# ramkp990/Truth_Recommendation_GNN

Measured on NVIDIA B200. Metric: message-passing edges/s (train step), higher is better.
Workload: dtype f32

## Files before the change

include/trg_b200.h:

```cpp
#ifndef TRG_B200_H
#define TRG_B200_H

#include <stddef.h>
#include <stdint.h>

#ifdef __cplusplus
extern "C" {
#endif

#define TRG_ABI_VERSION 4

enum { TRG_F32 = 0, TRG_BF16 = 1 };
enum {
  TRG_OK = 0,
  TRG_E_ARG = 1,
  TRG_E_WORKSPACE = 2,
  TRG_E_CUDA = 3,
  TRG_E_UNSUPPORTED = 4
};

int trg_abi_version(void);
const char* trg_last_error(void);
int64_t trg_launch_count(void);

size_t trg_csr_workspace_bytes(int64_t n_edges, int64_t n_key);
int trg_csr_build(const int64_t* other, const int64_t* key, int64_t n_edges, int64_t n_key,
                  int32_t* rowptr , int32_t* col , int32_t* eid ,
                  void* workspace, size_t workspace_bytes, void* stream);

size_t trg_select_range_workspace_bytes(int64_t n);
int trg_select_range(const int64_t* key, const int64_t* other, int64_t n, int64_t lo, int64_t hi,
                     int64_t capacity, int64_t pad_key, int64_t pad_other,
                     int64_t* key_out , int64_t* other_out ,
                     int32_t* count_out , void* workspace, size_t workspace_bytes, void* stream);

typedef struct {
  const int32_t* vrowptr;
  const int32_t* vinfo;
  int64_t n_vrows;
  const int32_t* long_rows;
  const int32_t* long_ptr;
  int64_t n_long;
  float* partial;
} trg_long_rows;

int trg_sage_agg_fwd(const int32_t* rowptr, const int32_t* col, const void* x_src,
                     int64_t n_dst, int32_t feat, int dtype,
                     void* mean_out , float* inv_deg_out ,
                     const trg_long_rows* long_rows , void* stream);

int trg_sage_agg_bwd(const int32_t* rowptr_t, const int32_t* col_t, const float* inv_deg,
                     const void* g_mean, int64_t n_src, int32_t feat, int dtype,
                     void* g_src_out , int out_dtype, int accumulate,
                     const void* relu_of, const trg_long_rows* long_rows ,
                     void* stream);

int trg_gather_wsum(const int32_t* rowptr, const int32_t* col, const int32_t* eid,
                    const float* coef, const float* scale, const void* x,
                    int64_t n_rows, int32_t feat, int dtype, void* out, int out_dtype, int accumulate,
                    const void* relu_of, const trg_long_rows* long_rows , void* stream);

int trg_rows_finish(const void* in, int in_dtype, const float* row_scale, const void* add,
                    const void* relu_of, int64_t n_rows, int32_t feat, int dtype, void* out, void* stream);

int trg_peer_reduce_rows(const void* const* parts, int32_t n_peers, int64_t row0, int in_dtype,
                         const float* row_scale, const void* add, const void* relu_of, int64_t n_rows,
                         int32_t feat, int dtype, void* out, int32_t ctas_per_sm, void* stream);

size_t trg_edge_bce_workspace_bytes(int64_t n_users);
int trg_edge_bce_fwd(const int32_t* rowptr_u, const int32_t* col_p, const int32_t* eid,
                     const int64_t* neg_p, const void* u, const void* p,
                     int64_t n_users, int64_t n_edges, int32_t hidden, int dtype,
                     const float* wbar , float* loss_out,
                     float* c_pos, float* c_neg, void* g_u,
                     void* workspace, size_t workspace_bytes, void* stream);

int trg_edge_anchor_loss(const int32_t* rowptr, const int32_t* col, const int32_t* eid,
                         const void* anchor, const void* gathered, int64_t n_rows,
                         int64_t n_edges_scale, int32_t hidden, int dtype, int label,
                         const float* wbar, float* loss_out, float* coef_out, void* g_anchor,
                         int accumulate, int relu_gate, void* workspace, size_t workspace_bytes,
                         void* stream);

typedef struct {
  const void* a;
  const void* w;
  int32_t k;
  float alpha;
} trg_proj_term;
size_t trg_sage_proj_workspace_bytes(int32_t k_total, int32_t hidden, int dtype);
int trg_sage_proj_fwd(const trg_proj_term* terms , int32_t n_terms,
                      const float* bias ,
                      int64_t n_rows, int32_t hidden, int dtype, int relu,
                      void* out ,
                      void* workspace, size_t workspace_bytes, void* stream);

typedef struct {
  const void* w;
  int32_t k;
  float alpha;
  const float* row_scale;
  void* d_a;
} trg_proj_bwd_term;
int trg_sage_proj_bwd_input(const void* dz, const trg_proj_bwd_term* terms , int32_t n_terms,
                            int64_t n_rows, int32_t hidden, int dtype,
                            void* workspace, size_t workspace_bytes, void* stream);

typedef struct {
  const void* a;
  int32_t k;
  float alpha;
  void* d_w;
} trg_proj_dw_term;
size_t trg_sage_proj_dw_workspace_bytes(void);
int trg_sage_proj_bwd_weight(const void* dz, const trg_proj_dw_term* terms , int32_t n_terms,
                             float* d_bias ,
                             int64_t n_rows, int32_t hidden, int dtype,
                             void* workspace, size_t workspace_bytes, void* stream);

size_t trg_score_topk_workspace_bytes(int64_t n_query, int64_t n_cat, int32_t hidden, int32_t k);
int trg_score_topk(const void* q , const void* cat ,
                   int64_t n_query, int64_t n_cat, int32_t hidden, int dtype, int32_t k,
                   int64_t id_offset, float* vals_out , int64_t* ids_out ,
                   void* workspace, size_t workspace_bytes, void* stream);
int trg_score_topk_excluding(const void* q , const void* cat ,
                             int64_t n_query, int64_t n_cat, int32_t hidden, int dtype, int32_t k,
                             int64_t id_offset, const int32_t* excl_rowptr ,
                             const int32_t* excl_ids , const int64_t* query_rows ,
                             float* vals_out , int64_t* ids_out ,
                             void* workspace, size_t workspace_bytes, void* stream);
int trg_topk_merge(const float* vals_in , const int64_t* ids_in,
                   int64_t n_query, int32_t n_lists, int32_t k_in, int32_t k_out,
                   float* vals_out, int64_t* ids_out, void* stream);

#ifdef __cplusplus
}
#endif
#endif
```

truth_recommendation_gnn_b200/_lib.py:

```python
from __future__ import annotations

import ctypes
import os

import torch

_HERE = os.path.dirname(os.path.abspath(__file__))
LIB_PATH = os.path.join(_HERE, "lib", "libtrg_b200.so")

TRG_F32, TRG_BF16 = 0, 1
ABI_VERSION = 4

_vp, _i64, _i32, _sz, _int = ctypes.c_void_p, ctypes.c_int64, ctypes.c_int32, ctypes.c_size_t, ctypes.c_int


class TrgProjTerm(ctypes.Structure):
    _fields_ = [("a", _vp), ("w", _vp), ("k", _i32), ("alpha", ctypes.c_float)]


class TrgLongRows(ctypes.Structure):
    _fields_ = [("vrowptr", _vp), ("vinfo", _vp), ("n_vrows", _i64), ("long_rows", _vp), ("long_ptr", _vp),
                ("n_long", _i64), ("partial", _vp)]


class TrgProjBwdTerm(ctypes.Structure):
    _fields_ = [("w", _vp), ("k", _i32), ("alpha", ctypes.c_float), ("row_scale", _vp), ("d_a", _vp)]


class TrgProjDwTerm(ctypes.Structure):
    _fields_ = [("a", _vp), ("k", _i32), ("alpha", ctypes.c_float), ("d_w", _vp)]


SIGNATURES = {
    "trg_abi_version": (_int, []),
    "trg_last_error": (ctypes.c_char_p, []),
    "trg_launch_count": (_i64, []),
    "trg_csr_workspace_bytes": (_sz, [_i64, _i64]),
    "trg_csr_build": (_int, [_vp, _vp, _i64, _i64, _vp, _vp, _vp, _vp, _sz, _vp]),
    "trg_select_range_workspace_bytes": (_sz, [_i64]),
    "trg_select_range": (_int, [_vp, _vp, _i64, _i64, _i64, _i64, _i64, _i64, _vp, _vp, _vp, _vp, _sz, _vp]),
    "trg_sage_agg_fwd": (_int, [_vp, _vp, _vp, _i64, _i32, _int, _vp, _vp, ctypes.POINTER(TrgLongRows), _vp]),
    "trg_sage_agg_bwd": (_int, [_vp, _vp, _vp, _vp, _i64, _i32, _int, _vp, _int, _int, _vp,
                                ctypes.POINTER(TrgLongRows), _vp]),
    "trg_gather_wsum": (_int, [_vp, _vp, _vp, _vp, _vp, _vp, _i64, _i32, _int, _vp, _int, _int, _vp,
                               ctypes.POINTER(TrgLongRows), _vp]),
    "trg_rows_finish": (_int, [_vp, _int, _vp, _vp, _vp, _i64, _i32, _int, _vp, _vp]),
    "trg_peer_reduce_rows": (_int, [_vp, _i32, _i64, _int, _vp, _vp, _vp, _i64, _i32, _int, _vp, _i32, _vp]),
    "trg_edge_bce_workspace_bytes": (_sz, [_i64]),
    "trg_edge_bce_fwd": (_int, [_vp, _vp, _vp, _vp, _vp, _vp, _i64, _i64, _i32, _int, _vp, _vp,
                                _vp, _vp, _vp, _vp, _sz, _vp]),
    "trg_edge_anchor_loss": (_int, [_vp, _vp, _vp, _vp, _vp, _i64, _i64, _i32, _int, _int, _vp, _vp, _vp,
                                    _vp, _int, _int, _vp, _sz, _vp]),
    "trg_sage_proj_workspace_bytes": (_sz, [_i32, _i32, _int]),
    "trg_sage_proj_fwd": (_int, [ctypes.POINTER(TrgProjTerm), _i32, _vp, _i64, _i32, _int, _int, _vp,
                                 _vp, _sz, _vp]),
    "trg_sage_proj_bwd_input": (_int, [_vp, ctypes.POINTER(TrgProjBwdTerm), _i32, _i64, _i32, _int,
                                       _vp, _sz, _vp]),
    "trg_sage_proj_dw_workspace_bytes": (_sz, []),
    "trg_sage_proj_bwd_weight": (_int, [_vp, ctypes.POINTER(TrgProjDwTerm), _i32, _vp, _i64, _i32, _int,
                                        _vp, _sz, _vp]),
    "trg_score_topk_workspace_bytes": (_sz, [_i64, _i64, _i32, _i32]),
    "trg_score_topk": (_int, [_vp, _vp, _i64, _i64, _i32, _int, _i32, _i64, _vp, _vp, _vp, _sz, _vp]),
    "trg_score_topk_excluding": (_int, [_vp, _vp, _i64, _i64, _i32, _int, _i32, _i64, _vp, _vp, _vp, _vp, _vp,
                                        _vp, _sz, _vp]),
    "trg_topk_merge": (_int, [_vp, _vp, _i64, _i32, _i32, _i32, _vp, _vp, _vp]),
}

_lib = None


class TrgError(RuntimeError):
    pass


def load():
    global _lib
    if _lib is None:
        if not os.path.exists(LIB_PATH):
            raise TrgError(
                f"{LIB_PATH} is missing: build it with `python -m truth_recommendation_gnn_b200.build` "
                "(nvcc, sm_100a). There is no CPU or PyTorch fallback for the hot path.")
        lib = ctypes.CDLL(LIB_PATH)
        for name, (res, args) in SIGNATURES.items():
            fn = getattr(lib, name)
            fn.restype, fn.argtypes = res, args
        if lib.trg_abi_version() != ABI_VERSION:
            raise TrgError("libtrg_b200.so ABI version mismatch; rebuild")
        _lib = lib
    return _lib


def check(rc: int, what: str):
    if rc != 0:
        raise TrgError(f"{what} failed (rc={rc}): {load().trg_last_error().decode()}")


def ptr(t):
    if t is None:
        return None
    if not t.is_cuda:
        raise TrgError("truth_recommendation_gnn_b200 runs on CUDA (sm_100a) tensors only; got a "
                       f"{t.device} tensor. There is no CPU fallback.")
    if not t.is_contiguous():
        raise TrgError("non-contiguous tensor passed to the C ABI")
    return t.data_ptr()


def stream():
    return torch.cuda.current_stream().cuda_stream


def dtype_code(dt: torch.dtype) -> int:
    if dt == torch.float32:
        return TRG_F32
    if dt == torch.bfloat16:
        return TRG_BF16
    raise TrgError(f"unsupported dtype {dt}: the hot path computes in fp32 or bf16 (fp32 accumulate)")


class Profiler:

    def __init__(self):
        self.enabled = False
        self.records = []

    def reset(self):
        self.records = []

    def summary(self):
        out = {}
        for name, nbytes, s, e in self.records:
            d = out.setdefault(name, dict(calls=0, ms=0.0, bytes=0))
            d["calls"] += 1
            d["ms"] += s.elapsed_time(e)
            d["bytes"] += int(nbytes)
        return out


PROF = Profiler()


def call(name, nbytes, fn, *args):
    if PROF.enabled:
        s, e = torch.cuda.Event(enable_timing=True), torch.cuda.Event(enable_timing=True)
        s.record()
        rc = fn(*args)
        e.record()
        PROF.records.append((name, nbytes, s, e))
    else:
        rc = fn(*args)
    check(rc, name)


def launch_count() -> int:
    return int(load().trg_launch_count())
```

truth_recommendation_gnn_b200/csrc/csr_build.cu:

```cuda
#include <algorithm>
#include <cstdio>

#include "common.cuh"

namespace trg {
namespace {

constexpr int kThreads = 256;
constexpr int kItems = 16;
constexpr int kTile = kThreads * kItems;
constexpr int kWarps = kThreads / 32;
constexpr int kRadix = 256;

template <int NWARPS>
__device__ __forceinline__ int block_exclusive_scan(int v, int* warp_sums, int& total) {
  const int lane = threadIdx.x & 31, w = threadIdx.x >> 5;
  int inc = v;
#pragma unroll
  for (int o = 1; o < 32; o <<= 1) {
    int t = __shfl_up_sync(0xffffffffu, inc, o);
    if (lane >= o) inc += t;
  }
  if (lane == 31) warp_sums[w] = inc;
  __syncthreads();
  int ws = (lane < NWARPS) ? warp_sums[lane] : 0;
  int winc = ws;
#pragma unroll
  for (int o = 1; o < NWARPS; o <<= 1) {
    int t = __shfl_up_sync(0xffffffffu, winc, o);
    if (lane >= o) winc += t;
  }
  const int wbase = __shfl_sync(0xffffffffu, winc - ws, w);
  total = __shfl_sync(0xffffffffu, winc, NWARPS - 1);
  __syncthreads();
  return wbase + inc - v;
}

__global__ void __launch_bounds__(kThreads) scan_tile_sums(const int* __restrict__ in, int64_t n,
                                                           int* __restrict__ tile_sums) {
  __shared__ int warp_sums[kWarps];
  const int64_t base = (int64_t)blockIdx.x * kTile;
  int s = 0;
#pragma unroll
  for (int i = 0; i < kItems; ++i) {
    int64_t idx = base + (int64_t)i * kThreads + threadIdx.x;
    if (idx < n) s += in[idx];
  }
  int total;
  block_exclusive_scan<kWarps>(s, warp_sums, total);
  if (threadIdx.x == 0) tile_sums[blockIdx.x] = total;
}

__global__ void __launch_bounds__(1024) scan_tile_offsets(int* __restrict__ tile_sums, int n_tiles) {
  __shared__ int warp_sums[32];
  int carry = 0;
  for (int base = 0; base < n_tiles; base += 1024) {
    int idx = base + threadIdx.x;
    int v = idx < n_tiles ? tile_sums[idx] : 0;
    int total;
    int ex = block_exclusive_scan<32>(v, warp_sums, total);
    if (idx < n_tiles) tile_sums[idx] = carry + ex;
    carry += total;
  }
}

__global__ void __launch_bounds__(kThreads) scan_apply(const int* in, int* out, int64_t n,
                                                       const int* __restrict__ tile_offsets) {
  __shared__ int warp_sums[kWarps];
  const int64_t base = (int64_t)blockIdx.x * kTile + (int64_t)threadIdx.x * kItems;
  int v[kItems];
  int s = 0;
#pragma unroll
  for (int i = 0; i < kItems; ++i) {
    v[i] = (base + i < n) ? in[base + i] : 0;
    s += v[i];
  }
  int total;
  int run = block_exclusive_scan<kWarps>(s, warp_sums, total) + tile_offsets[blockIdx.x];
#pragma unroll
  for (int i = 0; i < kItems; ++i) {
    if (base + i < n) out[base + i] = run;
    run += v[i];
  }
}

int exclusive_scan(const int* in, int* out, int64_t n, int* tile_sums, cudaStream_t st) {
  if (n <= 0) return TRG_OK;
  const int n_tiles = (int)ceil_div<int64_t>(n, kTile);
  scan_tile_sums<<<n_tiles, kThreads, 0, st>>>(in, n, tile_sums);
  scan_tile_offsets<<<1, 1024, 0, st>>>(tile_sums, n_tiles);
  scan_apply<<<n_tiles, kThreads, 0, st>>>(in, out, n, tile_sums);
  count_launch(3);
  TRG_LAUNCH_OK();
  return TRG_OK;
}

__global__ void __launch_bounds__(kThreads) count_keys(const long long* __restrict__ key, int64_t n,
                                                       long long n_key, int* __restrict__ deg) {
  int64_t i = (int64_t)blockIdx.x * blockDim.x + threadIdx.x;
  const int64_t stride = (int64_t)gridDim.x * blockDim.x;
  for (; i < n; i += stride) {
    const long long k = ldg_stream(key + i);
    if ((unsigned long long)k >= (unsigned long long)n_key) {
      printf("trg_csr_build: key %lld at edge %lld is outside [0, %lld)\n", k, (long long)i, n_key);
      __trap();
    }
    atomicAdd(&deg[(int)k], 1);
  }
}


__global__ void __launch_bounds__(kThreads) select_count(const long long* __restrict__ key, int64_t n,
                                                         long long lo, long long hi, int* __restrict__ tile_counts) {
  __shared__ int warp_sums[kWarps];
  const int64_t base = (int64_t)blockIdx.x * kTile;
  int c = 0;
#pragma unroll
  for (int i = 0; i < kItems; ++i) {
    const int64_t idx = base + (int64_t)i * kThreads + threadIdx.x;
    if (idx < n) {
      const long long k = ldg_stream(key + idx);
      c += (k >= lo && k < hi) ? 1 : 0;
    }
  }
  int total;
  block_exclusive_scan<kWarps>(c, warp_sums, total);
  if (threadIdx.x == 0) tile_counts[blockIdx.x] = total;
}

__global__ void __launch_bounds__(1024) select_offsets(int* __restrict__ tile_counts, int n_tiles,
                                                       long long capacity, int* __restrict__ count_out) {
  __shared__ int warp_sums[32];
  int carry = 0;
  for (int base = 0; base < n_tiles; base += 1024) {
    const int idx = base + threadIdx.x;
    const int v = idx < n_tiles ? tile_counts[idx] : 0;
    int total;
    const int ex = block_exclusive_scan<32>(v, warp_sums, total);
    if (idx < n_tiles) tile_counts[idx] = carry + ex;
    carry += total;
  }
  if (threadIdx.x == 0) {
    *count_out = carry;
    if ((long long)carry > capacity) {
      printf("trg_select_range: %d selected entries exceed the capacity %lld (negatives far from uniform? pass a larger "
             "capacity)\n", carry, capacity);
      __trap();
    }
  }
}

__global__ void __launch_bounds__(kThreads)
    select_scatter(const long long* __restrict__ key, const long long* __restrict__ other, int64_t n, long long lo,
                   long long hi, const int* __restrict__ tile_offsets, const int* __restrict__ count,
                   long long capacity, long long pad_key, long long pad_other, long long* __restrict__ key_out,
                   long long* __restrict__ other_out) {
  __shared__ int wtot[kWarps];
  const int lane = threadIdx.x & 31, w = threadIdx.x >> 5;
  const int64_t wbase = (int64_t)blockIdx.x * kTile + (int64_t)w * (kItems * 32);
  long long kv[kItems];
  unsigned sel[kItems];
  int mine = 0;
#pragma unroll
  for (int r = 0; r < kItems; ++r) {
    const int64_t idx = wbase + r * 32 + lane;
    kv[r] = idx < n ? ldg_stream(key + idx) : lo - 1;
    const bool in = kv[r] >= lo && kv[r] < hi;
    sel[r] = __ballot_sync(0xffffffffu, in);
    mine += __popc(sel[r]);
  }
  if (lane == 0) wtot[w] = mine;
  __syncthreads();
  int run = tile_offsets[blockIdx.x];
  for (int i = 0; i < w; ++i) run += wtot[i];
#pragma unroll
  for (int r = 0; r < kItems; ++r) {
    if ((sel[r] >> lane) & 1u) {
      const int dest = run + __popc(sel[r] & ((1u << lane) - 1u));
      if (dest < capacity) {
        key_out[dest] = kv[r] - lo;
        other_out[dest] = ldg_stream(other + wbase + r * 32 + lane);
      }
    }
    run += __popc(sel[r]);
  }
  const long long cnt = *count;
  for (long long i = cnt + (long long)blockIdx.x * kThreads + threadIdx.x; i < capacity;
       i += (long long)gridDim.x * kThreads) {
    key_out[i] = pad_key;
    other_out[i] = pad_other;
  }
}

__device__ __forceinline__ uint2 ldg_pair(const uint2* p) {
  uint2 r;
  asm volatile("ld.global.nc.L1::no_allocate.v2.u32 {%0,%1}, [%2];" : "=r"(r.x), "=r"(r.y) : "l"(p));
  return r;
}
template <bool FIRST>
__device__ __forceinline__ uint32_t load_key(const void* keys, int64_t idx) {
  if (FIRST) return (uint32_t)ldg_stream(reinterpret_cast<const long long*>(keys) + idx);
  return ldg_pair(reinterpret_cast<const uint2*>(keys) + idx).x;
}

template <bool FIRST>
__global__ void __launch_bounds__(kThreads) radix_hist(const void* __restrict__ keys, int64_t n,
                                                       int shift, int* __restrict__ hist,
                                                       int n_ctas) {
  __shared__ int h[kRadix];
  h[threadIdx.x] = 0;
  __syncthreads();
  const int64_t base = (int64_t)blockIdx.x * kTile;
#pragma unroll
  for (int i = 0; i < kItems; ++i) {
    int64_t idx = base + (int64_t)i * kThreads + threadIdx.x;
    if (idx < n) atomicAdd(&h[(load_key<FIRST>(keys, idx) >> shift) & (kRadix - 1)], 1);
  }
  __syncthreads();
  hist[(int64_t)threadIdx.x * n_ctas + blockIdx.x] = h[threadIdx.x];
}

template <bool FIRST, bool LAST>
__global__ void __launch_bounds__(kThreads)
    radix_scatter(const void* __restrict__ keys_in, int64_t n, int shift, const int* __restrict__ gbase,
                  int n_ctas, uint2* __restrict__ pairs_out, uint32_t* __restrict__ vals_out) {
  __shared__ int wcnt[kWarps][kRadix];
  __shared__ int sbase[kRadix];
  const int lane = threadIdx.x & 31, w = threadIdx.x >> 5;
#pragma unroll
  for (int i = 0; i < kWarps; ++i) wcnt[i][threadIdx.x] = 0;
  const int64_t wbase = (int64_t)blockIdx.x * kTile + (int64_t)w * (kItems * 32);

  uint32_t key[kItems], val[kItems];
#pragma unroll
  for (int r = 0; r < kItems; ++r) {
    int64_t idx = wbase + r * 32 + lane;
    bool valid = idx < n;
    if (FIRST) {
      key[r] = valid ? load_key<true>(keys_in, idx) : 0u;
      val[r] = (uint32_t)idx;
    } else {
      const uint2 kv = valid ? ldg_pair(reinterpret_cast<const uint2*>(keys_in) + idx) : make_uint2(0u, 0u);
      key[r] = kv.x;
      val[r] = kv.y;
    }
  }
  __syncthreads();

  int rank[kItems];
#pragma unroll
  for (int r = 0; r < kItems; ++r) {
    const bool valid = wbase + r * 32 + lane < n;
    const int d = valid ? (int)((key[r] >> shift) & (kRadix - 1)) : kRadix;
    const unsigned peers = __match_any_sync(0xffffffffu, d);
    const int prev = valid ? wcnt[w][d] : 0;
    __syncwarp();
    if (valid && lane == __ffs(peers) - 1) wcnt[w][d] = prev + __popc(peers);
    __syncwarp();
    rank[r] = prev + __popc(peers & ((1u << lane) - 1u));
  }
  __syncthreads();
  {
    int run = 0;
#pragma unroll
    for (int i = 0; i < kWarps; ++i) {
      int t = wcnt[i][threadIdx.x];
      wcnt[i][threadIdx.x] = run;
      run += t;
    }
    sbase[threadIdx.x] = gbase[(int64_t)threadIdx.x * n_ctas + blockIdx.x];
  }
  __syncthreads();
#pragma unroll
  for (int r = 0; r < kItems; ++r) {
    if (wbase + r * 32 + lane < n) {
      const int d = (int)((key[r] >> shift) & (kRadix - 1));
      const int dest = sbase[d] + wcnt[w][d] + rank[r];
      if (LAST)
        vals_out[dest] = val[r];
      else
        pairs_out[dest] = make_uint2(key[r], val[r]);
    }
  }
}

__global__ void __launch_bounds__(kThreads) gather_col(const long long* __restrict__ other,
                                                       const int* __restrict__ eid, int64_t n,
                                                       int* __restrict__ col) {
  int64_t i = (int64_t)blockIdx.x * blockDim.x + threadIdx.x;
  const int64_t stride = (int64_t)gridDim.x * blockDim.x;
  for (; i < n; i += stride) col[i] = (int)other[ldg_stream(eid + i)];
}

int num_passes(int64_t n_key) {
  int bits = 1;
  while (bits < 32 && ((int64_t)1 << bits) < n_key) ++bits;
  return (bits + 7) / 8;
}

struct Workspace {
  uint2* pairs[2];
  uint32_t* vals;
  int *hist, *tile_sums;
  size_t bytes;
};

Workspace carve(void* ws, int64_t e, int64_t n_key) {
  Workspace w;
  const size_t ebytes = align_up((size_t)(e > 0 ? e : 1) * 4, 256);
  const int64_t n_ctas = ceil_div<int64_t>(e > 0 ? e : 1, kTile);
  const size_t hist_bytes = align_up((size_t)kRadix * n_ctas * 4, 256);
  const int64_t scan_len = (int64_t)kRadix * n_ctas > n_key + 1 ? (int64_t)kRadix * n_ctas : n_key + 1;
  const size_t sums_bytes = align_up((size_t)ceil_div<int64_t>(scan_len, kTile) * 4 + 4, 256);
  char* p = reinterpret_cast<char*>(ws);
  w.pairs[0] = (uint2*)p; p += 2 * ebytes;
  w.pairs[1] = (uint2*)p; p += 2 * ebytes;
  w.vals = (uint32_t*)p; p += ebytes;
  w.hist = (int*)p; p += hist_bytes;
  w.tile_sums = (int*)p; p += sums_bytes;
  w.bytes = (size_t)(p - reinterpret_cast<char*>(ws));
  return w;
}

}
}

using namespace trg;

extern "C" size_t trg_csr_workspace_bytes(int64_t n_edges, int64_t n_key) {
  if (n_edges < 0 || n_key < 0) return 0;
  return carve(nullptr, n_edges, n_key).bytes;
}

extern "C" int trg_csr_build(const int64_t* other, const int64_t* key, int64_t e, int64_t n_key,
                             int32_t* rowptr, int32_t* col, int32_t* eid, void* workspace,
                             size_t workspace_bytes, void* stream) {
  cudaStream_t st = reinterpret_cast<cudaStream_t>(stream);
  TRG_CHECK_ARG(e >= 0 && n_key >= 0, "trg_csr_build: negative size");
  TRG_CHECK_ARG(e < ((int64_t)1 << 31) && n_key < ((int64_t)1 << 31) - 1,
                "trg_csr_build: n_edges=%lld / n_key=%lld exceed int32 CSR range", (long long)e,
                (long long)n_key);
  TRG_CHECK_ARG(rowptr != nullptr, "trg_csr_build: rowptr is NULL");
  TRG_CHECK_ARG(e == 0 || (key != nullptr && (col == nullptr || other != nullptr)),
                "trg_csr_build: NULL edge arrays with n_edges > 0");
  TRG_CHECK_ARG(e == 0 || n_key > 0, "trg_csr_build: edges present but n_key == 0");
  Workspace w = carve(workspace, e, n_key);
  if (workspace == nullptr || workspace_bytes < w.bytes) {
    set_error("trg_csr_build: workspace %zu < required %zu", workspace_bytes, w.bytes);
    return TRG_E_WORKSPACE;
  }
  TRG_CUDA(cudaMemsetAsync(rowptr, 0, (size_t)(n_key + 1) * sizeof(int32_t), st));
  if (e == 0) return TRG_OK;

  {
    int grid = (int)std::min<int64_t>(ceil_div<int64_t>(e, kThreads), (int64_t)kNumSMs * 16);
    count_keys<<<grid, kThreads, 0, st>>>((const long long*)key, e, (long long)n_key, rowptr);
    count_launch();
    TRG_LAUNCH_OK();
    int rc = exclusive_scan(rowptr, rowptr, n_key + 1, w.tile_sums, st);
    if (rc) return rc;
  }
  if (col == nullptr && eid == nullptr) return TRG_OK;

  const int passes = num_passes(n_key);
  const int n_ctas = (int)ceil_div<int64_t>(e, kTile);
  const void* kin = key;
  const uint32_t* vin = nullptr;
  for (int p = 0; p < passes; ++p) {
    const bool first = p == 0, last = p == passes - 1;
    const int shift = 8 * p;
    uint2* kout = w.pairs[p & 1];
    uint32_t* vout = eid ? (uint32_t*)eid : w.vals;
    if (first)
      radix_hist<true><<<n_ctas, kThreads, 0, st>>>(kin, e, shift, w.hist, n_ctas);
    else
      radix_hist<false><<<n_ctas, kThreads, 0, st>>>(kin, e, shift, w.hist, n_ctas);
    count_launch();
    TRG_LAUNCH_OK();
    int rc = exclusive_scan(w.hist, w.hist, (int64_t)kRadix * n_ctas, w.tile_sums, st);
    if (rc) return rc;
    if (first && last)
      radix_scatter<true, true><<<n_ctas, kThreads, 0, st>>>(kin, e, shift, w.hist, n_ctas, kout, vout);
    else if (first)
      radix_scatter<true, false><<<n_ctas, kThreads, 0, st>>>(kin, e, shift, w.hist, n_ctas, kout, vout);
    else if (last)
      radix_scatter<false, true><<<n_ctas, kThreads, 0, st>>>(kin, e, shift, w.hist, n_ctas, kout, vout);
    else
      radix_scatter<false, false><<<n_ctas, kThreads, 0, st>>>(kin, e, shift, w.hist, n_ctas, kout, vout);
    count_launch();
    TRG_LAUNCH_OK();
    kin = kout;
    vin = vout;
  }
  if (col != nullptr) {
    int grid = (int)std::min<int64_t>(ceil_div<int64_t>(e, kThreads), (int64_t)kNumSMs * 16);
    gather_col<<<grid, kThreads, 0, st>>>((const long long*)other, (const int*)vin, e, col);
    count_launch();
    TRG_LAUNCH_OK();
  }
  return TRG_OK;
}

extern "C" size_t trg_select_range_workspace_bytes(int64_t n) {
  if (n < 0) return 0;
  return align_up((size_t)(ceil_div<int64_t>(n > 0 ? n : 1, kTile) + 1) * 4, 256);
}

extern "C" int trg_select_range(const int64_t* key, const int64_t* other, int64_t n, int64_t lo, int64_t hi,
                                int64_t capacity, int64_t pad_key, int64_t pad_other, int64_t* key_out,
                                int64_t* other_out, int32_t* count_out, void* workspace, size_t workspace_bytes,
                                void* stream) {
  cudaStream_t st = reinterpret_cast<cudaStream_t>(stream);
  TRG_CHECK_ARG(n >= 0 && capacity >= 0 && lo <= hi, "trg_select_range: bad sizes");
  TRG_CHECK_ARG(n < ((int64_t)1 << 31) && capacity < ((int64_t)1 << 31), "trg_select_range: sizes exceed int32 range");
  TRG_CHECK_ARG(count_out && (capacity == 0 || (key_out && other_out)), "trg_select_range: NULL outputs");
  TRG_CHECK_ARG(n == 0 || (key && other), "trg_select_range: NULL inputs with n > 0");
  if (workspace == nullptr || workspace_bytes < trg_select_range_workspace_bytes(n)) {
    set_error("trg_select_range: workspace %zu < required %zu", workspace_bytes, trg_select_range_workspace_bytes(n));
    return TRG_E_WORKSPACE;
  }
  int* tile_counts = reinterpret_cast<int*>(workspace);
  const int n_tiles = (int)ceil_div<int64_t>(n > 0 ? n : 1, kTile);
  select_count<<<n_tiles, kThreads, 0, st>>>((const long long*)key, n, lo, hi, tile_counts);
  select_offsets<<<1, 1024, 0, st>>>(tile_counts, n_tiles, capacity, count_out);
  select_scatter<<<n_tiles, kThreads, 0, st>>>((const long long*)key, (const long long*)other, n, lo, hi, tile_counts,
                                               count_out, capacity, pad_key, pad_other, (long long*)key_out,
                                               (long long*)other_out);
  count_launch(3);
  TRG_LAUNCH_OK();
  return TRG_OK;
}
```

truth_recommendation_gnn_b200/csrc/edge_bce.cu:

```cuda
#include <cstdlib>

#include "common.cuh"

namespace trg {
namespace {

constexpr int kThreads = 256;

struct BceArgs {
  const int* rowptr;
  const int* col_p;
  const int* eid;
  const long long* neg_p;
  const void* u;
  const void* p;
  const float* wbar;
  float* c_pos;
  float* c_neg;
  void* g_u;
  double* partials;
  int64_t n_users;
  float inv_e;
  int row_vecs;
  int label;
  int accumulate;
  int relu_gate;
};

__device__ __forceinline__ float softplus(float x) {
  return fmaxf(x, 0.f) + log1pf(expf(-fabsf(x)));
}
__device__ __forceinline__ float sigmoid(float x) {
  const float e = expf(-fabsf(x));
  return x >= 0.f ? __fdiv_rn(1.f, 1.f + e) : __fdiv_rn(e, 1.f + e);
}

template <typename T, int LPR, int VPL, int R, bool TWO>
__global__ void __launch_bounds__(kThreads, VPL == 1 ? 3 : 2) edge_bce(const BceArgs a) {
  constexpr int kVec = Elem<T>::kVec;
  constexpr int kUnroll = (LPR < 8 ? (LPR >= 4 ? 2 : 1) : (VPL == 1 ? 4 : 2)) * (TWO ? 1 : 2);
  static_assert(R < LPR, "row boundaries are held one per lane");
  __shared__ double red[2][kThreads / 32];
  const int lane = threadIdx.x & 31;
  const int gl = lane & (LPR - 1);
  const unsigned gmask = LPR == 32 ? 0xffffffffu : (((1u << LPR) - 1u) << (lane & ~(LPR - 1)));
  const int64_t r0 = ((int64_t)blockIdx.x * (kThreads / LPR) + threadIdx.x / LPR) * R;
  const bool want_grad = a.g_u != nullptr;
  float sp_sum = 0.f, sn_sum = 0.f;

  if (r0 < a.n_users) {
    const int nr = (int)((a.n_users - r0) < (int64_t)R ? (a.n_users - r0) : (int64_t)R);
    const int my_ptr = ldg_stream(a.rowptr + r0 + min(gl, nr));
    const int e_end = __shfl_sync(gmask, my_ptr, nr, LPR);
    int e0 = __shfl_sync(gmask, my_ptr, 0, LPR);
    const size_t row_bytes = (size_t)a.row_vecs * 16;
    const char* pb = reinterpret_cast<const char*>(a.p);
    const char* ub = reinterpret_cast<const char*>(a.u);
    const float wbar = __ldg(a.wbar);

    bool act[VPL];
    float uf[VPL][kVec], ga[VPL][kVec];
    uint4 u_nxt[VPL];
#pragma unroll
    for (int i = 0; i < VPL; ++i) {
      act[i] = gl + i * LPR < a.row_vecs;
#pragma unroll
      for (int k = 0; k < kVec; ++k) uf[i][k] = ga[i][k] = 0.f;
      u_nxt[i] = make_uint4(0, 0, 0, 0);
      if (act[i]) {
        Elem<T>::unpack(ldg_row(ub + (size_t)r0 * row_bytes + (size_t)(gl + i * LPR) * 16), uf[i]);
        if (nr > 1) u_nxt[i] = ldg_row(ub + (size_t)(r0 + 1) * row_bytes + (size_t)(gl + i * LPR) * 16);
      }
    }
    int cur = 0;
    int cur_end = __shfl_sync(gmask, my_ptr, 1, LPR);

    auto flush = [&]() {
      if (want_grad) {
        char* ob = reinterpret_cast<char*>(a.g_u) + (size_t)(r0 + cur) * row_bytes;
#pragma unroll
        for (int i = 0; i < VPL; ++i)
          if (act[i]) {
            if (!TWO && a.accumulate) {
              float f[kVec];
              Elem<T>::unpack(*reinterpret_cast<const uint4*>(ob + (size_t)(gl + i * LPR) * 16), f);
#pragma unroll
              for (int k = 0; k < kVec; ++k) ga[i][k] += f[k];
            }
            if (!TWO && a.relu_gate) {
#pragma unroll
              for (int k = 0; k < kVec; ++k) ga[i][k] = uf[i][k] > 0.f ? ga[i][k] : 0.f;
            }
            stg_stream(ob + (size_t)(gl + i * LPR) * 16, Elem<T>::pack(ga[i]));
          }
      }
      ++cur;
      cur_end = __shfl_sync(gmask, my_ptr, min(cur + 1, nr), LPR);
#pragma unroll
      for (int i = 0; i < VPL; ++i) {
        Elem<T>::unpack(u_nxt[i], uf[i]);
#pragma unroll
        for (int k = 0; k < kVec; ++k) ga[i][k] = 0.f;
        if (act[i] && cur + 1 < nr)
          u_nxt[i] = ldg_row(ub + (size_t)(r0 + cur + 1) * row_bytes + (size_t)(gl + i * LPR) * 16);
      }
    };

    auto load_idx = [&](int e, int& cp, int& id) {
      cp = 0; id = 0;
      if (e < e_end) {
        cp = ldg_stream(a.col_p + e);
        id = a.eid ? ldg_stream(a.eid + e) : e;
      }
    };
    int cp_cur, id_cur, cn_cur = 0, cp_nxt, id_nxt;
    load_idx(e0 + gl, cp_cur, id_cur);
    if (TWO && e0 + gl < e_end) cn_cur = (int)ldg_stream(a.neg_p + id_cur);
    load_idx(e0 + LPR + gl, cp_nxt, id_nxt);

    while (e0 < e_end) {
      const int cnt = min(LPR, e_end - e0);
      int cn_nxt = 0;
      if (TWO && e0 + LPR + gl < e_end) cn_nxt = (int)ldg_stream(a.neg_p + id_nxt);
      int cp_nn, id_nn;
      load_idx(e0 + 2 * LPR + gl, cp_nn, id_nn);
      float my_cpos = 0.f, my_cneg = 0.f;

      int t = 0;
      while (t < cnt) {
        while (e0 + t >= cur_end) flush();
        const int bsz = min(min(kUnroll, cnt - t), cur_end - (e0 + t));
        uint4 vp[kUnroll][VPL], vn[kUnroll][VPL];
#pragma unroll
        for (int q = 0; q < kUnroll; ++q) {
          const int cpq = __shfl_sync(gmask, cp_cur, t + q, LPR);
          const int cnq = __shfl_sync(gmask, cn_cur, t + q, LPR);
          if (q < bsz) {
#pragma unroll
            for (int i = 0; i < VPL; ++i)
              if (act[i]) {
                vp[q][i] = ldg_row(pb + (size_t)cpq * row_bytes + (size_t)(gl + i * LPR) * 16);
                if (TWO) vn[q][i] = ldg_row(pb + (size_t)cnq * row_bytes + (size_t)(gl + i * LPR) * 16);
              }
          }
        }
        constexpr int NV = TWO ? 2 * kUnroll : kUnroll;
        static_assert(LPR >= NV, "transpose-reduce needs at least one lane per value");
        float v[NV];
#pragma unroll
        for (int q = 0; q < kUnroll; ++q) {
          float dp = 0.f, dn = 0.f;
          if (q < bsz) {
#pragma unroll
            for (int i = 0; i < VPL; ++i) {
              if (act[i]) {
                float fp[kVec], fn[kVec];
                Elem<T>::unpack(vp[q][i], fp);
                if (TWO) Elem<T>::unpack(vn[q][i], fn);
#pragma unroll
                for (int k = 0; k < kVec; ++k) {
                  dp = fmaf(uf[i][k], fp[k], dp);
                  if (TWO) dn = fmaf(uf[i][k], fn[k], dn);
                }
              }
            }
          }
          if (TWO) {
            v[2 * q] = dp;
            v[2 * q + 1] = dn;
          } else {
            v[q] = dp;
          }
        }
        int nv = NV;
#pragma unroll
        for (int o = LPR / 2; o > 0; o >>= 1) {
          if (nv > 1) {
            nv >>= 1;
#pragma unroll
            for (int i = 0; i < NV / 2; ++i) {
              if (i < nv) {
                const bool hi = (gl & o) != 0;
                const float send = hi ? v[i] : v[i + nv];
                const float keep = hi ? v[i + nv] : v[i];
                v[i] = keep + __shfl_xor_sync(gmask, send, o, LPR);
              }
            }
          } else {
            v[0] += __shfl_xor_sync(gmask, v[0], o, LPR);
          }
        }
        constexpr int kLanesPerVal = LPR / NV;
        const int j = gl / kLanesPerVal;
        const bool is_neg = TWO ? (j & 1) : (a.label == 0);
        const float z = is_neg ? v[0] : -v[0];
        const float spv = softplus(z);
        if ((gl % kLanesPerVal) == 0 && (TWO ? (j >> 1) : j) < bsz) {
          if (is_neg) sn_sum += spv; else sp_sum += spv;
        }
        if (want_grad) {
          const float coef = (is_neg ? 1.f : -wbar) * sigmoid(z) * a.inv_e;
#pragma unroll
          for (int q = 0; q < kUnroll; ++q) {
            const float cpos = __shfl_sync(gmask, coef, (TWO ? 2 * q : q) * kLanesPerVal, LPR);
            const float cneg = TWO ? __shfl_sync(gmask, coef, (2 * q + 1) * kLanesPerVal, LPR) : 0.f;
            if (q < bsz) {
              if (gl == t + q) {
                my_cpos = cpos;
                my_cneg = cneg;
              }
#pragma unroll
              for (int i = 0; i < VPL; ++i)
                if (act[i]) {
                  float fp[kVec], fn[kVec];
                  Elem<T>::unpack(vp[q][i], fp);
                  if (TWO) Elem<T>::unpack(vn[q][i], fn);
#pragma unroll
                  for (int k = 0; k < kVec; ++k)
                    ga[i][k] = TWO ? fmaf(cpos, fp[k], fmaf(cneg, fn[k], ga[i][k])) : fmaf(cpos, fp[k], ga[i][k]);
                }
            }
          }
        }
        t += bsz;
      }
      if (want_grad && e0 + gl < e_end) {
        a.c_pos[id_cur] = my_cpos;
        if (TWO) a.c_neg[id_cur] = my_cneg;
      }
      e0 += LPR;
      cp_cur = cp_nxt; id_cur = id_nxt; cn_cur = cn_nxt;
      cp_nxt = cp_nn; id_nxt = id_nn;
    }
    while (cur < nr) flush();
  }

  double dsp = sp_sum, dsn = sn_sum;
#pragma unroll
  for (int o = 16; o > 0; o >>= 1) {
    dsp += __shfl_xor_sync(0xffffffffu, dsp, o);
    dsn += __shfl_xor_sync(0xffffffffu, dsn, o);
  }
  if (lane == 0) {
    red[0][threadIdx.x >> 5] = dsp;
    red[1][threadIdx.x >> 5] = dsn;
  }
  __syncthreads();
  if (threadIdx.x == 0) {
    double s0 = 0, s1 = 0;
#pragma unroll
    for (int w = 0; w < kThreads / 32; ++w) {
      s0 += red[0][w];
      s1 += red[1][w];
    }
    a.partials[2 * (size_t)blockIdx.x] = s0;
    a.partials[2 * (size_t)blockIdx.x + 1] = s1;
  }
}

__device__ __forceinline__ void cp_async16(uint32_t dst, const void* src) {
  asm volatile("cp.async.cg.shared.global [%0], [%1], 16;" ::"r"(dst), "l"(src) : "memory");
}
__device__ __forceinline__ void cp_async_commit() { asm volatile("cp.async.commit_group;" ::: "memory"); }
template <int N>
__device__ __forceinline__ void cp_async_wait() {
  asm volatile("cp.async.wait_group %0;" ::"n"(N) : "memory");
}
__device__ __forceinline__ uint4 lds128_bce(uint32_t addr) {
  uint4 v;
  asm volatile("ld.shared.v4.u32 {%0,%1,%2,%3}, [%4];" : "=r"(v.x), "=r"(v.y), "=r"(v.z), "=r"(v.w) : "r"(addr) : "memory");
  return v;
}

constexpr int kRingG = 8;
constexpr int kRingS = 16;
constexpr int kRingBytes = (kThreads / 32) * kRingS * 512;

template <typename T>
__global__ void __launch_bounds__(kThreads, 3) edge_anchor_ring(const BceArgs a) {
  constexpr int kVec = Elem<T>::kVec;
  constexpr int R = 4, G = kRingG, S = kRingS;
  constexpr unsigned full = 0xffffffffu;
  extern __shared__ __align__(16) unsigned char ring_raw[];
  __shared__ double red[2][kThreads / 32];
  const int lane = threadIdx.x & 31, warp = threadIdx.x >> 5;
  const uint32_t ring_a = static_cast<uint32_t>(__cvta_generic_to_shared(ring_raw)) +
                          (uint32_t)(warp * S * 512 + lane * 16);
  const int64_t r0 = ((int64_t)blockIdx.x * (kThreads / 32) + warp) * R;
  const bool want_grad = a.g_u != nullptr;
  float s_sum = 0.f;

  if (r0 < a.n_users) {
    const int nr = (int)((a.n_users - r0) < (int64_t)R ? (a.n_users - r0) : (int64_t)R);
    const int my_ptr = ldg_stream(a.rowptr + r0 + min(lane, nr));
    const int e_end = __shfl_sync(full, my_ptr, nr);
    const int e_beg = __shfl_sync(full, my_ptr, 0);
    const char* pb = reinterpret_cast<const char*>(a.p);
    const char* ub = reinterpret_cast<const char*>(a.u);
    const float wbar = __ldg(a.wbar);
    const bool is_neg = a.label == 0;

    float uf[kVec], ga[kVec];
    uint4 u_nxt = make_uint4(0, 0, 0, 0);
#pragma unroll
    for (int k = 0; k < kVec; ++k) ga[k] = 0.f;
    Elem<T>::unpack(ldg_row(ub + (size_t)r0 * 512 + (size_t)lane * 16), uf);
    if (nr > 1) u_nxt = ldg_row(ub + (size_t)(r0 + 1) * 512 + (size_t)lane * 16);
    int cur = 0;
    int cur_end = __shfl_sync(full, my_ptr, 1);

    auto flush = [&]() {
      if (want_grad) {
        char* ob = reinterpret_cast<char*>(a.g_u) + (size_t)(r0 + cur) * 512 + (size_t)lane * 16;
        if (a.accumulate) {
          float f[kVec];
          Elem<T>::unpack(*reinterpret_cast<const uint4*>(ob), f);
#pragma unroll
          for (int k = 0; k < kVec; ++k) ga[k] += f[k];
        }
        if (a.relu_gate) {
#pragma unroll
          for (int k = 0; k < kVec; ++k) ga[k] = uf[k] > 0.f ? ga[k] : 0.f;
        }
        stg_stream(ob, Elem<T>::pack(ga));
      }
      ++cur;
      cur_end = __shfl_sync(full, my_ptr, min(cur + 1, nr));
      Elem<T>::unpack(u_nxt, uf);
#pragma unroll
      for (int k = 0; k < kVec; ++k) ga[k] = 0.f;
      if (cur + 1 < nr) u_nxt = ldg_row(ub + (size_t)(r0 + cur + 1) * 512 + (size_t)lane * 16);
    };
    auto load_id = [&](int ebase) -> int {
      const int e = ebase + lane;
      return (lane < G && e < e_end) ? ldg_stream(a.col_p + e) : 0;
    };
    auto issue = [&](int ebase, int ids, int slot0) {
#pragma unroll
      for (int q = 0; q < G; ++q) {
        const int rid = __shfl_sync(full, ids, q);
        if (ebase + q < e_end)
          cp_async16(ring_a + (uint32_t)(((slot0 + q) & (S - 1)) * 512), pb + (size_t)rid * 512 + (size_t)lane * 16);
      }
      cp_async_commit();
    };

    {
      const int id0 = load_id(e_beg), id1 = load_id(e_beg + G);
      issue(e_beg, id0, 0);
      issue(e_beg + G, id1, G);
    }
    int nid = load_id(e_beg + 2 * G);
    int slot = 0;
    for (int e_base = e_beg; e_base < e_end; e_base += G) {
      const int cnt = min(G, e_end - e_base);
      int my_id = 0;
      if (want_grad && lane < cnt) my_id = a.eid ? ldg_stream(a.eid + e_base + lane) : e_base + lane;
      cp_async_wait<1>();
      __syncwarp();
      float my_c = 0.f;
      int t = 0;
      while (t < cnt) {
        while (e_base + t >= cur_end) flush();
        const int bsz = min(cnt - t, cur_end - (e_base + t));
        uint4 vp[G];
        float v[G];
#pragma unroll
        for (int q = 0; q < G; ++q) {
          float dp = 0.f;
          if (q < bsz) {
            vp[q] = lds128_bce(ring_a + (uint32_t)(((slot + t + q) & (S - 1)) * 512));
            float fp[kVec];
            Elem<T>::unpack(vp[q], fp);
#pragma unroll
            for (int k = 0; k < kVec; ++k) dp = fmaf(uf[k], fp[k], dp);
          }
          v[q] = dp;
        }
        int nv = G;
#pragma unroll
        for (int o = 16; o > 0; o >>= 1) {
          if (nv > 1) {
            nv >>= 1;
#pragma unroll
            for (int i = 0; i < G / 2; ++i) {
              if (i < nv) {
                const bool hi = (lane & o) != 0;
                const float send = hi ? v[i] : v[i + nv];
                const float keep = hi ? v[i + nv] : v[i];
                v[i] = keep + __shfl_xor_sync(full, send, o);
              }
            }
          } else {
            v[0] += __shfl_xor_sync(full, v[0], o);
          }
        }
        constexpr int kLanesPerVal = 32 / G;
        const int j = lane / kLanesPerVal;
        const float z = is_neg ? v[0] : -v[0];
        const float spv = softplus(z);
        if ((lane % kLanesPerVal) == 0 && j < bsz) s_sum += spv;
        if (want_grad) {
          const float coef = (is_neg ? 1.f : -wbar) * sigmoid(z) * a.inv_e;
#pragma unroll
          for (int q = 0; q < G; ++q) {
            const float cq = __shfl_sync(full, coef, q * kLanesPerVal);
            if (q < bsz) {
              if (lane == t + q) my_c = cq;
              float fp[kVec];
              Elem<T>::unpack(vp[q], fp);
#pragma unroll
              for (int k = 0; k < kVec; ++k) ga[k] = fmaf(cq, fp[k], ga[k]);
            }
          }
        }
        t += bsz;
      }
      if (want_grad && lane < cnt) a.c_pos[my_id] = my_c;
      __syncwarp();
      const int nid_next = load_id(e_base + 3 * G);
      issue(e_base + 2 * G, nid, slot);
      nid = nid_next;
      slot = (slot + G) & (S - 1);
    }
    while (cur < nr) flush();
    cp_async_wait<0>();
  }

  double dsum = s_sum;
#pragma unroll
  for (int o = 16; o > 0; o >>= 1) dsum += __shfl_xor_sync(0xffffffffu, dsum, o);
  if (lane == 0) red[0][warp] = dsum;
  __syncthreads();
  if (threadIdx.x == 0) {
    double s0 = 0;
#pragma unroll
    for (int w = 0; w < kThreads / 32; ++w) s0 += red[0][w];
    const bool neg = a.label == 0;
    a.partials[2 * (size_t)blockIdx.x] = neg ? 0.0 : s0;
    a.partials[2 * (size_t)blockIdx.x + 1] = neg ? s0 : 0.0;
  }
}

__global__ void __launch_bounds__(1024) edge_bce_finish(const double* __restrict__ partials,
                                                        int64_t n_parts, const float* wbar,
                                                        double n_edges, float* loss_out) {
  __shared__ double red[2][32];
  double s0 = 0, s1 = 0;
  for (int64_t i = threadIdx.x; i < n_parts; i += 1024) {
    s0 += partials[2 * i];
    s1 += partials[2 * i + 1];
  }
#pragma unroll
  for (int o = 16; o > 0; o >>= 1) {
    s0 += __shfl_xor_sync(0xffffffffu, s0, o);
    s1 += __shfl_xor_sync(0xffffffffu, s1, o);
  }
  if ((threadIdx.x & 31) == 0) {
    red[0][threadIdx.x >> 5] = s0;
    red[1][threadIdx.x >> 5] = s1;
  }
  __syncthreads();
  if (threadIdx.x == 0) {
    s0 = s1 = 0;
    for (int w = 0; w < 32; ++w) {
      s0 += red[0][w];
      s1 += red[1][w];
    }
    const float pos_loss = (float)(s0 / n_edges);
    const float neg_loss = (float)(s1 / n_edges);
    loss_out[0] = __ldg(wbar) * pos_loss + neg_loss;
  }
}

template <typename T, bool TWO>
int launch_bce(BceArgs& a, int64_t* n_blocks_out, cudaStream_t st, bool dry) {
  const int rv = a.row_vecs;
#define TRG_BCE_CASE(LPR, VPL, R)                                                     \
  {                                                                                   \
    const int64_t grid = ceil_div<int64_t>(a.n_users, (int64_t)(kThreads / LPR) * R); \
    *n_blocks_out = grid;                                                             \
    if (!dry) edge_bce<T, LPR, VPL, R, TWO><<<(unsigned)grid, kThreads, 0, st>>>(a);  \
  }
  if (rv <= 2) TRG_BCE_CASE(2, 1, 1)
  else if (rv <= 4) TRG_BCE_CASE(4, 1, 2)
  else if (rv <= 8) TRG_BCE_CASE(8, 1, 4)
  else if (rv <= 16) TRG_BCE_CASE(16, 1, 4)
  else if (rv <= 32) TRG_BCE_CASE(32, 1, 4)
  else if (rv <= 64) TRG_BCE_CASE(32, 2, 4)
  else {
    set_error("trg_edge_bce_fwd: rows wider than 1024 bytes are not supported (row_vecs=%d)", rv);
    return TRG_E_UNSUPPORTED;
  }
#undef TRG_BCE_CASE
  return TRG_OK;
}

}
}

using namespace trg;

static bool anchor_ring_off() { return debug_env_int("TRG_K4_RING", 1) == 0; }

extern "C" size_t trg_edge_bce_workspace_bytes(int64_t n_users) {
  if (n_users < 0) return 0;
  return align_up((size_t)(ceil_div<int64_t>(n_users, 8) + 1) * 16, 256);
}

extern "C" int trg_edge_bce_fwd(const int32_t* rowptr_u, const int32_t* col_p, const int32_t* eid,
                                const int64_t* neg_p, const void* u, const void* p, int64_t n_users,
                                int64_t n_edges, int32_t hidden, int dtype, const float* wbar,
                                float* loss_out, float* c_pos, float* c_neg, void* g_u,
                                void* workspace, size_t workspace_bytes, void* stream) {
  cudaStream_t st = reinterpret_cast<cudaStream_t>(stream);
  TRG_CHECK_ARG(n_users >= 0 && n_edges >= 0, "trg_edge_bce_fwd: negative size");
  TRG_CHECK_ARG(loss_out && wbar, "trg_edge_bce_fwd: NULL loss_out/wbar");
  TRG_CHECK_ARG((c_pos == nullptr) == (g_u == nullptr) && (c_neg == nullptr) == (g_u == nullptr),
                "trg_edge_bce_fwd: c_pos, c_neg and g_u must be all NULL or all non-NULL");
  TRG_CHECK_ARG(n_users == 0 || (rowptr_u && u && p), "trg_edge_bce_fwd: NULL rowptr / tables");
  TRG_CHECK_ARG(((uintptr_t)u | (uintptr_t)p | (uintptr_t)g_u) % 16 == 0,
                "trg_edge_bce_fwd: tables must be 16-byte aligned");
  const int es = dtype == TRG_BF16 ? 2 : 4;
  TRG_CHECK_ARG(dtype == TRG_F32 || dtype == TRG_BF16, "trg_edge_bce_fwd: unknown dtype %d", dtype);
  TRG_CHECK_ARG(hidden > 0 && (hidden * es) % 16 == 0,
                "trg_edge_bce_fwd: row width %d x %d bytes is not a multiple of 16 bytes", hidden, es);
  if (workspace == nullptr || workspace_bytes < trg_edge_bce_workspace_bytes(n_users)) {
    set_error("trg_edge_bce_fwd: workspace %zu < required %zu", workspace_bytes,
              trg_edge_bce_workspace_bytes(n_users));
    return TRG_E_WORKSPACE;
  }
  BceArgs a{};
  a.rowptr = rowptr_u; a.col_p = col_p; a.eid = eid; a.neg_p = (const long long*)neg_p;
  a.u = u; a.p = p; a.wbar = wbar; a.c_pos = c_pos; a.c_neg = c_neg; a.g_u = g_u;
  a.partials = reinterpret_cast<double*>(workspace);
  a.n_users = n_users;
  a.inv_e = n_edges > 0 ? (float)(1.0 / (double)n_edges) : 0.f;
  a.row_vecs = hidden * es / 16;
  int64_t n_blocks = 0;
  if (n_users > 0) {
    int rc = dtype == TRG_F32 ? launch_bce<float, true>(a, &n_blocks, st, false)
                              : launch_bce<__nv_bfloat16, true>(a, &n_blocks, st, false);
    if (rc) return rc;
    count_launch();
    TRG_LAUNCH_OK();
  }
  edge_bce_finish<<<1, 1024, 0, st>>>(a.partials, n_blocks, wbar, (double)n_edges, loss_out);
  count_launch();
  TRG_LAUNCH_OK();
  return TRG_OK;
}

extern "C" int trg_edge_anchor_loss(const int32_t* rowptr, const int32_t* col, const int32_t* eid,
                                    const void* anchor, const void* gathered, int64_t n_rows,
                                    int64_t n_edges_scale, int32_t hidden, int dtype, int label,
                                    const float* wbar, float* loss_out, float* coef_out, void* g_anchor,
                                    int accumulate, int relu_gate, void* workspace, size_t workspace_bytes,
                                    void* stream) {
  cudaStream_t st = reinterpret_cast<cudaStream_t>(stream);
  TRG_CHECK_ARG(n_rows >= 0 && n_edges_scale >= 0, "trg_edge_anchor_loss: negative size");
  TRG_CHECK_ARG(loss_out && wbar, "trg_edge_anchor_loss: NULL loss_out/wbar");
  TRG_CHECK_ARG((coef_out == nullptr) == (g_anchor == nullptr),
                "trg_edge_anchor_loss: coef_out and g_anchor must be both NULL or both non-NULL");
  TRG_CHECK_ARG(n_rows == 0 || (rowptr && anchor), "trg_edge_anchor_loss: NULL rowptr / anchor table");
  TRG_CHECK_ARG(((uintptr_t)anchor | (uintptr_t)gathered | (uintptr_t)g_anchor) % 16 == 0,
                "trg_edge_anchor_loss: tables must be 16-byte aligned");
  TRG_CHECK_ARG(dtype == TRG_F32 || dtype == TRG_BF16, "trg_edge_anchor_loss: unknown dtype %d", dtype);
  const int es = dtype == TRG_BF16 ? 2 : 4;
  TRG_CHECK_ARG(hidden > 0 && (hidden * es) % 16 == 0,
                "trg_edge_anchor_loss: row width %d x %d bytes is not a multiple of 16 bytes", hidden, es);
  if (workspace == nullptr || workspace_bytes < trg_edge_bce_workspace_bytes(n_rows)) {
    set_error("trg_edge_anchor_loss: workspace %zu < required %zu", workspace_bytes,
              trg_edge_bce_workspace_bytes(n_rows));
    return TRG_E_WORKSPACE;
  }
  BceArgs a{};
  a.rowptr = rowptr; a.col_p = col; a.eid = eid; a.neg_p = nullptr;
  a.u = anchor; a.p = gathered; a.wbar = wbar; a.c_pos = coef_out; a.c_neg = nullptr; a.g_u = g_anchor;
  a.partials = reinterpret_cast<double*>(workspace);
  a.n_users = n_rows;
  a.inv_e = n_edges_scale > 0 ? (float)(1.0 / (double)n_edges_scale) : 0.f;
  a.row_vecs = hidden * es / 16;
  a.label = label ? 1 : 0;
  a.accumulate = accumulate ? 1 : 0;
  a.relu_gate = relu_gate ? 1 : 0;
  int64_t n_blocks = 0;
  if (n_rows > 0 && a.row_vecs == 32 && !anchor_ring_off()) {
    n_blocks = ceil_div<int64_t>(n_rows, (int64_t)(kThreads / 32) * 4);
    static SmemAttrState attr_f32, attr_bf16;
    if (dtype == TRG_F32) {
      TRG_CUDA(ensure_dyn_smem(edge_anchor_ring<float>, kRingBytes, attr_f32));
      edge_anchor_ring<float><<<(unsigned)n_blocks, kThreads, kRingBytes, st>>>(a);
    } else {
      TRG_CUDA(ensure_dyn_smem(edge_anchor_ring<__nv_bfloat16>, kRingBytes, attr_bf16));
      edge_anchor_ring<__nv_bfloat16><<<(unsigned)n_blocks, kThreads, kRingBytes, st>>>(a);
    }
    count_launch();
    TRG_LAUNCH_OK();
  } else if (n_rows > 0) {
    int rc = dtype == TRG_F32 ? launch_bce<float, false>(a, &n_blocks, st, false)
                              : launch_bce<__nv_bfloat16, false>(a, &n_blocks, st, false);
    if (rc) return rc;
    count_launch();
    TRG_LAUNCH_OK();
  }
  edge_bce_finish<<<1, 1024, 0, st>>>(a.partials, n_blocks, wbar, (double)n_edges_scale, loss_out);
  count_launch();
  TRG_LAUNCH_OK();
  return TRG_OK;
}
```

truth_recommendation_gnn_b200/functional.py:

```python
from __future__ import annotations

import ctypes

import torch

from . import _lib
from .graph import CSR, RelationGraph, build_csr


def _long_rows_arg(csr: CSR, feat: int, dev, elem_size: int = 4):
    lr = csr.long_rows() if feat * elem_size >= 80 else None
    if lr is None:
        return None, None
    partial = torch.empty(lr.n_slots, feat, dtype=torch.float32, device=dev)
    s = _lib.TrgLongRows(_lib.ptr(lr.vrowptr), _lib.ptr(lr.vinfo), int(lr.vinfo.numel()), _lib.ptr(lr.long_rows),
                         _lib.ptr(lr.long_ptr), int(lr.long_rows.numel()), _lib.ptr(partial))
    return ctypes.byref(s), (s, partial)


def _check_rows(x: torch.Tensor, what: str):
    es = x.element_size()
    if x.dim() != 2 or (x.size(1) * es) % 16 != 0:
        raise _lib.TrgError(f"{what}: rows must be a multiple of 16 bytes (got shape {tuple(x.shape)}, "
                            f"{x.dtype}); pad the feature width (the reference pads to 64, inference.py:401-404)")


def sage_agg_fwd(csr: CSR, x_src: torch.Tensor, want_inv_deg: bool = True):
    lib = _lib.load()
    _check_rows(x_src, "sage_agg_fwd")
    x_src = x_src.contiguous()
    out = torch.empty(csr.n_rows, x_src.size(1), dtype=x_src.dtype, device=x_src.device)
    inv_deg = torch.empty(csr.n_rows, dtype=torch.float32, device=x_src.device) if want_inv_deg else None
    if csr.n_rows:
        rb = x_src.size(1) * x_src.element_size()
        nbytes = csr.n_edges * (rb + 4) + 4 * (csr.n_rows + 1) + csr.n_rows * rb
        lr, keep = _long_rows_arg(csr, x_src.size(1), x_src.device, x_src.element_size())
        _lib.call("trg_sage_agg_fwd", nbytes, lib.trg_sage_agg_fwd,
                  _lib.ptr(csr.rowptr), _lib.ptr(csr.col), _lib.ptr(x_src), csr.n_rows, x_src.size(1),
                  _lib.dtype_code(x_src.dtype), _lib.ptr(out), _lib.ptr(inv_deg), lr, _lib.stream())
    return out, inv_deg


def _check_epilogue(out, relu_of, n_rows, x, who, out_dtype=None):
    for t, what, dt in ((out, "out", out_dtype or x.dtype), (relu_of, "relu_of", x.dtype)):
        if t is not None and (t.shape != (n_rows, x.size(1)) or t.dtype != dt or not t.is_contiguous()
                              or t.device != x.device):
            raise _lib.TrgError(f"{who}: {what} must be a contiguous [{n_rows}, {x.size(1)}] {dt} tensor")


def _out_dtype(x, out, out_dtype):
    if out_dtype is None:
        out_dtype = out.dtype if out is not None else x.dtype
    if out_dtype != x.dtype and not (x.dtype == torch.bfloat16 and out_dtype == torch.float32):
        raise _lib.TrgError(f"output dtype {out_dtype} is not supported for a {x.dtype} table")
    return out_dtype


def sage_agg_bwd(csr_t: CSR, inv_deg, g_mean: torch.Tensor, out=None, accumulate=False, relu_of=None,
                 out_dtype=None):
    lib = _lib.load()
    g_mean = g_mean.contiguous()
    _check_rows(g_mean, "sage_agg_bwd")
    out_dtype = _out_dtype(g_mean, out, out_dtype)
    _check_epilogue(out, relu_of, csr_t.n_rows, g_mean, "sage_agg_bwd", out_dtype)
    if out is None:
        out = torch.empty(csr_t.n_rows, g_mean.size(1), dtype=out_dtype, device=g_mean.device)
        accumulate = False
    if csr_t.n_rows:
        rb = g_mean.size(1) * g_mean.element_size()
        ob = g_mean.size(1) * out.element_size()
        nbytes = (csr_t.n_edges * (rb + 4) + 4 * (csr_t.n_rows + 1)
                  + csr_t.n_rows * (ob * (1 + bool(accumulate)) + rb * (relu_of is not None))
                  + (4 * csr_t.n_cols if inv_deg is not None else 0))
        lr, keep = _long_rows_arg(csr_t, g_mean.size(1), g_mean.device, g_mean.element_size())
        _lib.call("trg_sage_agg_bwd", nbytes, lib.trg_sage_agg_bwd,
                  _lib.ptr(csr_t.rowptr), _lib.ptr(csr_t.col), _lib.ptr(inv_deg), _lib.ptr(g_mean),
                  csr_t.n_rows, g_mean.size(1), _lib.dtype_code(g_mean.dtype), _lib.ptr(out),
                  _lib.dtype_code(out_dtype), 1 if accumulate else 0, _lib.ptr(relu_of), lr, _lib.stream())
    return out


class SageAggFn(torch.autograd.Function):

    @staticmethod
    def forward(ctx, x_src, rel: RelationGraph, grad_prescaled: bool = False):
        want_inv = rel.inv_deg is None
        mean, inv_deg = sage_agg_fwd(rel.fwd, x_src, want_inv_deg=want_inv)
        if want_inv:
            rel.inv_deg = inv_deg
        ctx.rel = rel
        ctx.grad_prescaled = grad_prescaled
        return mean

    @staticmethod
    def backward(ctx, g_mean):
        if not ctx.needs_input_grad[0]:
            return None, None, None
        rel = ctx.rel
        return sage_agg_bwd(rel.bwd, None if ctx.grad_prescaled else rel.inv_deg, g_mean), None, None


def sage_mean_aggregate(x_src: torch.Tensor, rel: RelationGraph, grad_prescaled: bool = False) -> torch.Tensor:
    return SageAggFn.apply(x_src, rel, grad_prescaled)


def gather_wsum(csr: CSR, coef, x: torch.Tensor, scale=None, out=None, accumulate=False, relu_of=None,
                out_dtype=None):
    lib = _lib.load()
    x = x.contiguous()
    _check_rows(x, "gather_wsum")
    out_dtype = _out_dtype(x, out, out_dtype)
    _check_epilogue(out, relu_of, csr.n_rows, x, "gather_wsum", out_dtype)
    if out is None:
        out = torch.empty(csr.n_rows, x.size(1), dtype=out_dtype, device=x.device)
        accumulate = False
    if csr.n_rows:
        rb = x.size(1) * x.element_size()
        ob = x.size(1) * out.element_size()
        nbytes = (csr.n_edges * (rb + 12) + 4 * (csr.n_rows + 1)
                  + csr.n_rows * (ob * (1 + bool(accumulate)) + rb * (relu_of is not None)))
        lr, keep = _long_rows_arg(csr, x.size(1), x.device, x.element_size())
        _lib.call("trg_gather_wsum", nbytes, lib.trg_gather_wsum,
                  _lib.ptr(csr.rowptr), _lib.ptr(csr.col), _lib.ptr(csr.eid), _lib.ptr(coef),
                  _lib.ptr(scale), _lib.ptr(x), csr.n_rows, x.size(1), _lib.dtype_code(x.dtype),
                  _lib.ptr(out), _lib.dtype_code(out_dtype), 1 if accumulate else 0, _lib.ptr(relu_of), lr,
                  _lib.stream())
    return out


def rows_finish(x, dtype, row_scale=None, add=None, relu_of=None, out=None):
    lib = _lib.load()
    x = x.contiguous()
    n, feat = x.shape
    if x.dtype != dtype and x.dtype != torch.float32:
        raise _lib.TrgError(f"rows_finish: input must be {dtype} or float32, got {x.dtype}")
    for t, what in ((add, "add"), (relu_of, "relu_of"), (out, "out")):
        if t is not None and (t.shape != x.shape or t.dtype != dtype or not t.is_contiguous()):
            raise _lib.TrgError(f"rows_finish: {what} must be a contiguous [{n}, {feat}] {dtype} tensor")
    if out is None:
        out = torch.empty(n, feat, dtype=dtype, device=x.device)
    _check_rows(out, "rows_finish")
    rs = row_scale.float().contiguous() if row_scale is not None else None
    es = out.element_size()
    nbytes = n * feat * (x.element_size() + es * (1 + (add is not None) + (relu_of is not None)))
    _lib.call("trg_rows_finish", nbytes, lib.trg_rows_finish, _lib.ptr(x), _lib.dtype_code(x.dtype), _lib.ptr(rs),
              _lib.ptr(add), _lib.ptr(relu_of), n, feat, _lib.dtype_code(dtype), _lib.ptr(out), _lib.stream())
    return out


def peer_reduce_rows(parts, row0, n_rows, dtype, row_scale=None, add=None, relu_of=None, ctas_per_sm=0):
    import ctypes
    lib = _lib.load()
    feat = parts[0].size(1)
    for t in parts:
        if t.dtype != parts[0].dtype or t.size(1) != feat or t.size(0) < row0 + n_rows or not t.is_contiguous():
            raise _lib.TrgError("peer_reduce_rows: partial tables must be contiguous, of one dtype and width, and "
                                "hold rows [row0, row0 + n_rows)")
    if parts[0].dtype != dtype and parts[0].dtype != torch.float32:
        raise _lib.TrgError(f"peer_reduce_rows: partial tables must be {dtype} or float32")
    for t, what in ((add, "add"), (relu_of, "relu_of")):
        if t is not None and (tuple(t.shape) != (n_rows, feat) or t.dtype != dtype or not t.is_contiguous()):
            raise _lib.TrgError(f"peer_reduce_rows: {what} must be a contiguous [{n_rows}, {feat}] {dtype} tensor")
    out = torch.empty(n_rows, feat, dtype=dtype, device=parts[0].device)
    _check_rows(out, "peer_reduce_rows")
    rs = row_scale.float().contiguous() if row_scale is not None else None
    ptrs = (ctypes.c_void_p * len(parts))(*[_lib.ptr(t) for t in parts])
    nbytes = n_rows * feat * (len(parts) * parts[0].element_size()
                              + out.element_size() * (1 + (add is not None) + (relu_of is not None)))
    _lib.call("trg_peer_reduce_rows", nbytes, lib.trg_peer_reduce_rows, ptrs, len(parts), row0,
              _lib.dtype_code(parts[0].dtype), _lib.ptr(rs), _lib.ptr(add), _lib.ptr(relu_of), n_rows, feat,
              _lib.dtype_code(dtype), _lib.ptr(out), ctas_per_sm, _lib.stream())
    return out


class LinkStructure:

    def __init__(self, train_edge_index, interaction_type_tensor, num_users, num_posts):
        pos_u, pos_p = train_edge_index[0], train_edge_index[1]
        self.train_edge_index = train_edge_index
        self.num_users, self.num_posts = int(num_users), int(num_posts)
        self.n_edges = int(pos_u.numel())
        self.by_user = build_csr(pos_p, pos_u, self.num_users, self.num_posts)
        self.by_post = build_csr(pos_u, pos_p, self.num_posts, self.num_users, validate=False)
        self._by_post_u = None
        self._user_of_u = None
        if self.n_edges:
            w = interaction_type_tensor[pos_p + num_users].float()
            self.wbar = w.mean().reshape(1).contiguous()
        else:
            self.wbar = torch.full((1,), float("nan"), device=pos_u.device)


    @property
    def by_post_u(self) -> CSR:
        if self._by_post_u is None:
            bu, bp = self.by_user, self.by_post
            inv = torch.empty(self.n_edges, dtype=torch.int32, device=bu.eid.device)
            inv[bu.eid.long()] = torch.arange(self.n_edges, dtype=torch.int32, device=bu.eid.device)
            self._by_post_u = CSR(bp.rowptr, bp.col, inv[bp.eid.long()].contiguous(), bp.n_rows, bp.n_cols, bp._long)
        return self._by_post_u

    @property
    def user_of_u(self) -> torch.Tensor:
        if self._user_of_u is None:
            rp = self.by_user.rowptr.long()
            self._user_of_u = torch.repeat_interleave(
                torch.arange(self.num_users, device=rp.device), rp[1:] - rp[:-1]).contiguous()
        return self._user_of_u


_LINK_CACHE: dict = {}


def link_structure(train_edge_index, interaction_type_tensor, num_users, num_posts) -> LinkStructure:
    key = (train_edge_index.data_ptr(), tuple(train_edge_index.shape), train_edge_index._version,
           interaction_type_tensor.data_ptr(), interaction_type_tensor._version, int(num_users),
           int(num_posts))
    s = _LINK_CACHE.get(key)
    if s is None:
        if len(_LINK_CACHE) > 8:
            _LINK_CACHE.clear()
        s = LinkStructure(train_edge_index, interaction_type_tensor, num_users, num_posts)
        s._keepalive = interaction_type_tensor
        _LINK_CACHE[key] = s
    return s


def edge_bce_fwd(ls: LinkStructure, user_emb, post_emb, neg_p, want_grad: bool):
    lib = _lib.load()
    _check_rows(user_emb, "edge_bce_fwd")
    if user_emb.dtype != post_emb.dtype or user_emb.size(1) != post_emb.size(1):
        raise _lib.TrgError("user and post embeddings must share dtype and width")
    if neg_p.dtype != torch.int64 or neg_p.numel() != ls.n_edges:
        raise _lib.TrgError("neg_p must be int64 with one entry per positive edge (train_gnn.py:272)")
    user_emb, post_emb, neg_p = user_emb.contiguous(), post_emb.contiguous(), neg_p.contiguous()
    dev = user_emb.device
    loss = torch.empty(1, dtype=torch.float32, device=dev)
    c_pos = c_neg = g_u = None
    if want_grad:
        c_pos = torch.empty(ls.n_edges, dtype=torch.float32, device=dev)
        c_neg = torch.empty(ls.n_edges, dtype=torch.float32, device=dev)
        g_u = torch.empty_like(user_emb)
    ws_bytes = int(lib.trg_edge_bce_workspace_bytes(ls.num_users))
    ws = torch.empty(ws_bytes, dtype=torch.uint8, device=dev)
    e = ls.n_edges
    e_scale = int(getattr(ls, "n_edges_scale", e))
    rb = user_emb.size(1) * user_emb.element_size()
    nbytes = e * (2 * rb + 16 + (8 if want_grad else 0)) + ls.num_users * (rb * (2 if want_grad else 1) + 4)
    _lib.call("trg_edge_bce_fwd", nbytes, lib.trg_edge_bce_fwd,
              _lib.ptr(ls.by_user.rowptr), _lib.ptr(ls.by_user.col) if e else None,
              _lib.ptr(ls.by_user.eid) if e else None, _lib.ptr(neg_p) if e else None,
              _lib.ptr(user_emb), _lib.ptr(post_emb), ls.num_users, e_scale, user_emb.size(1),
              _lib.dtype_code(user_emb.dtype), _lib.ptr(ls.wbar), _lib.ptr(loss), _lib.ptr(c_pos),
              _lib.ptr(c_neg), _lib.ptr(g_u), _lib.ptr(ws), ws_bytes, _lib.stream())
    return loss, c_pos, c_neg, g_u


def edge_anchor_loss(csr: CSR, anchor, gathered, n_edges_scale, label, wbar, want_grad, g_anchor=None,
                     relu_gate=False, coef_in_csr_order=False):
    lib = _lib.load()
    anchor, gathered = anchor.contiguous(), gathered.contiguous()
    _check_rows(anchor, "edge_anchor_loss")
    dev = anchor.device
    loss = torch.empty(1, dtype=torch.float32, device=dev)
    coef = None
    accumulate = g_anchor is not None
    if want_grad:
        coef = torch.empty(csr.n_edges, dtype=torch.float32, device=dev)
        if g_anchor is None:
            g_anchor = torch.empty_like(anchor)
    else:
        g_anchor = None
    ws_bytes = int(lib.trg_edge_bce_workspace_bytes(csr.n_rows))
    ws = torch.empty(ws_bytes, dtype=torch.uint8, device=dev)
    e = csr.n_edges
    rb = anchor.size(1) * anchor.element_size()
    nbytes = e * (rb + 12) + csr.n_rows * (rb * (2 if want_grad else 1) + 4)
    _lib.call("trg_edge_anchor_loss", nbytes, lib.trg_edge_anchor_loss,
              _lib.ptr(csr.rowptr), _lib.ptr(csr.col) if e else None,
              _lib.ptr(csr.eid) if (e and not coef_in_csr_order) else None,
              _lib.ptr(anchor), _lib.ptr(gathered), csr.n_rows, int(n_edges_scale), anchor.size(1),
              _lib.dtype_code(anchor.dtype), 1 if label else 0, _lib.ptr(wbar), _lib.ptr(loss), _lib.ptr(coef),
              _lib.ptr(g_anchor), 1 if (accumulate and want_grad) else 0,
              1 if (relu_gate and want_grad) else 0, _lib.ptr(ws), ws_bytes, _lib.stream())
    return loss, coef, g_anchor


class LinkBCEFn(torch.autograd.Function):

    @staticmethod
    def forward(ctx, user_emb, post_emb, neg_p, ls: LinkStructure):
        want = user_emb.requires_grad or post_emb.requires_grad
        if neg_p.dtype != torch.int64 or neg_p.numel() != ls.n_edges:
            raise _lib.TrgError("neg_p must be int64 with one entry per positive edge (train_gnn.py:272)")
        if getattr(ls, "eid_long", None) is None:
            ls.eid_long = ls.by_user.eid.long()
        e_scale = int(getattr(ls, "n_edges_scale", ls.n_edges))
        bu = ls.by_user
        ctx.neg_by_post = None
        if want and ls.n_edges:
            ctx.neg_by_post = build_csr(ls.train_edge_index[0], neg_p, ls.num_posts, ls.num_users, validate=False,
                                        per_step=True)
        col_neg = neg_p.index_select(0, ls.eid_long).int()
        neg_csr = CSR(bu.rowptr, col_neg, bu.eid, bu.n_rows, bu.n_cols)
        l_pos, c_pos, g_u = edge_anchor_loss(bu, user_emb, post_emb, e_scale, 1, ls.wbar, want, None)
        l_neg, c_neg, g_u = edge_anchor_loss(neg_csr, user_emb, post_emb, e_scale, 0, ls.wbar, want, g_u)
        ctx.ls = ls
        ctx.want = want
        if want:
            ctx.save_for_backward(user_emb, neg_p, c_pos, c_neg, g_u)
        return (l_pos + l_neg).reshape(())

    @staticmethod
    def backward(ctx, g):
        user_emb, neg_p, c_pos, c_neg, g_u = ctx.saved_tensors
        ls = ctx.ls
        g = g.reshape(1).float().contiguous()
        g_user = g_post = None
        if ctx.needs_input_grad[0]:
            g_user = g_u * g.to(g_u.dtype)
        if ctx.needs_input_grad[1]:
            g_post = gather_wsum(ls.by_post, c_pos, user_emb, scale=g)
            if ctx.neg_by_post is not None:
                gather_wsum(ctx.neg_by_post, c_neg, user_emb, scale=g, out=g_post, accumulate=True)
        return g_user, g_post, None, None


def link_bce_loss(user_emb, post_emb, train_edge_index, neg_p, interaction_type_tensor, num_users):
    ls = link_structure(train_edge_index, interaction_type_tensor, num_users, post_emb.size(0))
    return LinkBCEFn.apply(user_emb, post_emb, neg_p, ls)


def _proj_bytes(n, ks, hidden, es):
    return n * (sum(ks) + hidden) * es


def sage_proj_fwd(terms, bias, relu: bool):
    lib = _lib.load()
    a0 = terms[0][0]
    n, hidden = a0.size(0), terms[0][1].size(0)
    arr = (_lib.TrgProjTerm * len(terms))()
    keep = []
    for i, (a, w, alpha) in enumerate(terms):
        a, w = a.contiguous(), w.contiguous()
        if a.dtype != a0.dtype or w.dtype != a0.dtype:
            raise _lib.TrgError("projection operands must share one dtype")
        keep += [a, w]
        arr[i].a, arr[i].w, arr[i].k, arr[i].alpha = _lib.ptr(a), _lib.ptr(w), a.size(1), float(alpha)
    out = torch.empty(n, hidden, dtype=a0.dtype, device=a0.device)
    b = bias.float().contiguous() if bias is not None else None
    ktot = sum(t[0].size(1) for t in terms)
    code = _lib.dtype_code(a0.dtype)
    ws_bytes = int(lib.trg_sage_proj_workspace_bytes(ktot, hidden, code))
    ws = torch.empty(ws_bytes, dtype=torch.uint8, device=a0.device)
    _lib.call("trg_sage_proj_fwd", _proj_bytes(n, [t[0].size(1) for t in terms], hidden, a0.element_size()),
              lib.trg_sage_proj_fwd, arr, len(terms), _lib.ptr(b), n, hidden, code, 1 if relu else 0,
              _lib.ptr(out), _lib.ptr(ws), ws_bytes, _lib.stream())
    return out


def sage_proj_bwd_input(dz, terms):
    lib = _lib.load()
    dz = dz.contiguous()
    n, hidden = dz.shape
    arr = (_lib.TrgProjBwdTerm * len(terms))()
    outs, keep = [], []
    for i, (w, alpha, rs) in enumerate(terms):
        w = w.contiguous()
        if w.dtype != dz.dtype:
            raise _lib.TrgError("projection operands must share one dtype")
        d_a = torch.empty(n, w.size(1), dtype=dz.dtype, device=dz.device)
        rs = rs.float().contiguous() if rs is not None else None
        keep += [w, rs]
        outs.append(d_a)
        arr[i].w, arr[i].k, arr[i].alpha = _lib.ptr(w), w.size(1), float(alpha)
        arr[i].row_scale, arr[i].d_a = _lib.ptr(rs), _lib.ptr(d_a)
    ktot = sum(t[0].size(1) for t in terms)
    code = _lib.dtype_code(dz.dtype)
    ws_bytes = int(lib.trg_sage_proj_workspace_bytes(ktot, hidden, code))
    ws = torch.empty(ws_bytes, dtype=torch.uint8, device=dz.device)
    _lib.call("trg_sage_proj_bwd_input", n * (len(terms) * hidden + ktot) * dz.element_size(),
              lib.trg_sage_proj_bwd_input, _lib.ptr(dz), arr, len(terms), n, hidden, code,
              _lib.ptr(ws), ws_bytes, _lib.stream())
    return outs


class FusedProjFn(torch.autograd.Function):

    @staticmethod
    def forward(ctx, relu, alphas, row_scales, bias, *aw):
        n_t = len(aw) // 2
        a_list, w_list = aw[:n_t], aw[n_t:]
        out = sage_proj_fwd([(a, w, al) for a, w, al in zip(a_list, w_list, alphas)], bias, relu)
        ctx.relu, ctx.alphas, ctx.row_scales, ctx.n_t = relu, alphas, row_scales, n_t
        ctx.has_bias = bias is not None
        ctx.bias_dtype = bias.dtype if bias is not None else None
        ctx.save_for_backward(out, *a_list, *w_list)
        return out

    @staticmethod
    def backward(ctx, g):
        out, *rest = ctx.saved_tensors
        n_t = ctx.n_t
        a_list, w_list = rest[:n_t], rest[n_t:]
        g = g.contiguous()
        dz = torch.ops.aten.threshold_backward(g, out, 0) if ctx.relu else g
        need_a = [ctx.needs_input_grad[4 + t] for t in range(n_t)]
        need_w = [ctx.needs_input_grad[4 + n_t + t] for t in range(n_t)]
        d_a = [None] * n_t
        idx = [t for t in range(n_t) if need_a[t]]
        if idx:
            outs = sage_proj_bwd_input(dz, [(w_list[t], ctx.alphas[t], ctx.row_scales[t]) for t in idx])
            for t, o in zip(idx, outs):
                d_a[t] = o
        d_w = [None] * n_t
        widx = [t for t in range(n_t) if need_w[t]]
        want_b = ctx.has_bias and ctx.needs_input_grad[3]
        d_b = None
        if widx or want_b:
            outs, d_b = sage_proj_bwd_weight(dz, [(a_list[t], ctx.alphas[t]) for t in widx], want_b)
            for t, o in zip(widx, outs):
                d_w[t] = o
            if d_b is not None:
                d_b = d_b.to(ctx.bias_dtype)
        return (None, None, None, d_b, *d_a, *d_w)


def sage_proj_bwd_weight(dz, terms, want_bias: bool):
    lib = _lib.load()
    dz = dz.contiguous()
    n, hidden = dz.shape
    arr = (_lib.TrgProjDwTerm * max(len(terms), 1))()
    outs, keep = [], []
    for i, (a, alpha) in enumerate(terms):
        a = a.contiguous()
        d_w = torch.empty(hidden, a.size(1), dtype=dz.dtype, device=dz.device)
        keep.append(a)
        outs.append(d_w)
        arr[i].a, arr[i].k, arr[i].alpha, arr[i].d_w = _lib.ptr(a), a.size(1), float(alpha), _lib.ptr(d_w)
    db = torch.empty(hidden, dtype=torch.float32, device=dz.device) if want_bias else None
    ws_bytes = int(lib.trg_sage_proj_dw_workspace_bytes())
    ws = torch.empty(ws_bytes, dtype=torch.uint8, device=dz.device)
    ktot = sum(t[0].size(1) for t in terms)
    _lib.call("trg_sage_proj_bwd_weight", n * (hidden + ktot) * dz.element_size(),
              lib.trg_sage_proj_bwd_weight, _lib.ptr(dz), arr, len(terms), _lib.ptr(db), n, hidden,
              _lib.dtype_code(dz.dtype), _lib.ptr(ws), ws_bytes, _lib.stream())
    return outs, db


def fused_projection(terms, bias, relu=True, row_scales=None):
    a_list = [t[0] for t in terms]
    w_list = [t[1] for t in terms]
    alphas = tuple(float(t[2]) for t in terms)
    rs = tuple(row_scales) if row_scales is not None else (None,) * len(terms)
    return FusedProjFn.apply(relu, alphas, rs, bias, *a_list, *w_list)


def score_topk(q: torch.Tensor, cat: torch.Tensor, k: int, id_offset: int = 0, exclude=None, rows=None):
    lib = _lib.load()
    if q.dim() == 1:
        q = q.unsqueeze(0)
    q, cat = q.contiguous(), cat.contiguous()
    b, h = q.shape
    p = cat.size(0)
    kk = min(int(k), p)
    if exclude is None and rows is not None:
        raise ValueError("score_topk: rows selects exclusion rows and needs exclude")
    if exclude is not None:
        if rows is None:
            if b > exclude.num_rows:
                raise ValueError(f"score_topk: {b} queries but the exclusion index has {exclude.num_rows} rows; "
                                 "pass rows= to map queries to rows")
        else:
            if rows.dtype != torch.int64 or rows.dim() != 1 or rows.numel() != b:
                raise ValueError(f"score_topk: rows must be int64 [B={b}]")
            rows = rows.contiguous()
    vals = torch.empty(b, kk, dtype=torch.float32, device=q.device)
    ids = torch.empty(b, kk, dtype=torch.int64, device=q.device)
    if b == 0 or kk == 0:
        return vals, ids
    ws_bytes = int(lib.trg_score_topk_workspace_bytes(b, p, h, kk))
    ws = torch.empty(ws_bytes, dtype=torch.uint8, device=q.device)
    if exclude is None:
        _lib.call("trg_score_topk", 2 * b * p * h, lib.trg_score_topk,
                  _lib.ptr(q), _lib.ptr(cat), b, p, h, _lib.dtype_code(q.dtype), kk, int(id_offset),
                  _lib.ptr(vals), _lib.ptr(ids), _lib.ptr(ws), ws_bytes, _lib.stream())
    else:
        _lib.call("trg_score_topk_excluding", 2 * b * p * h, lib.trg_score_topk_excluding,
                  _lib.ptr(q), _lib.ptr(cat), b, p, h, _lib.dtype_code(q.dtype), kk, int(id_offset),
                  _lib.ptr(exclude.rowptr), _lib.ptr(exclude.ids if exclude.nnz else exclude.rowptr), _lib.ptr(rows),
                  _lib.ptr(vals), _lib.ptr(ids), _lib.ptr(ws), ws_bytes, _lib.stream())
    return vals, ids


def topk_merge(vals_in: torch.Tensor, ids_in: torch.Tensor, n_lists: int, k_out: int):
    lib = _lib.load()
    b = vals_in.size(0)
    k_in = vals_in.size(1) // n_lists
    vals = torch.empty(b, k_out, dtype=torch.float32, device=vals_in.device)
    ids = torch.empty(b, k_out, dtype=torch.int64, device=vals_in.device)
    _lib.check(lib.trg_topk_merge(_lib.ptr(vals_in.contiguous()), _lib.ptr(ids_in.contiguous()), b,
                                  n_lists, k_in, k_out, _lib.ptr(vals), _lib.ptr(ids), _lib.stream()),
               "trg_topk_merge")
    return vals, ids
```

truth_recommendation_gnn_b200/fused_step.py:

```python
from __future__ import annotations

import torch

from . import _lib
from .functional import (edge_anchor_loss, gather_wsum, link_structure, sage_agg_bwd, sage_agg_fwd,
                         sage_proj_bwd_input, sage_proj_bwd_weight, sage_proj_fwd)
from .graph import CSR, build_csr, relation_graph
from .nn import REL_DIRECT, REL_ENGAGE, REL_SOCIAL, StackedWeightedRGCN, WeightedRGCN


def _layers(model):
    if type(model) is StackedWeightedRGCN:
        return list(model.layers)
    if type(model) is WeightedRGCN:
        return [model]
    return None


def eligible(model, x_dict) -> bool:
    layers = _layers(model)
    if layers is None or not torch.is_grad_enabled():
        return False
    xu, xp = x_dict["user"], x_dict["post"]
    if not (xu.is_cuda and xp.is_cuda) or xu.requires_grad or xp.requires_grad or xu.dtype != xp.dtype:
        return False
    for layer in layers:
        for conv in (layer.msg_direct, layer.msg_social, layer.post_update):
            if conv.lin_l.bias is None:
                return False
    return all(p.requires_grad for p in model.parameters())


def _accum(param, grad):
    grad = grad.to(param.dtype)
    if param.grad is None:
        param.grad = grad
    else:
        param.grad.add_(grad)


def _agg(rel, x):
    want_inv = rel.inv_deg is None
    mean, inv_deg = sage_agg_fwd(rel.fwd, x, want_inv_deg=want_inv)
    if want_inv:
        rel.inv_deg = inv_deg
    return mean


@torch.no_grad()
def loss_and_grads(model, x_dict, edge_index_dict, train_edge_index, interaction_type_tensor, num_users,
                   neg_p, neg_ready=None):
    layers = _layers(model)
    if layers is None:
        raise _lib.TrgError("loss_and_grads: model must be WeightedRGCN or StackedWeightedRGCN")
    hu, hp = x_dict["user"].contiguous(), x_dict["post"].contiguous()
    n_u, n_p = hu.size(0), hp.size(0)
    rel_d = relation_graph(edge_index_dict[REL_DIRECT], n_p, n_u)
    rel_s = relation_graph(edge_index_dict[REL_SOCIAL], n_u, n_u)
    rel_e = relation_graph(edge_index_dict[REL_ENGAGE], n_u, n_p)

    saved = []
    for layer in layers:
        d, s, p = layer.msg_direct, layer.msg_social, layer.post_update
        for conv, (xs, xd) in ((d, (hp, hu)), (s, (hu, hu)), (p, (hu, hp))):
            conv.lin_l.materialize(xs.size(-1))
            conv.lin_r.materialize(xd.size(-1))
        wd, ws = float(layer.w_direct), float(layer.w_social)
        mean_d, mean_s, mean_e = _agg(rel_d, hp), _agg(rel_s, hu), _agg(rel_e, hu)
        w_root = wd * d.lin_r.weight + ws * s.lin_r.weight
        b_user = wd * d.lin_l.bias + ws * s.lin_l.bias
        hu_n = sage_proj_fwd([(mean_d, d.lin_l.weight, wd), (mean_s, s.lin_l.weight, ws), (hu, w_root, 1.0)],
                             b_user, True)
        hp_n = sage_proj_fwd([(mean_e, p.lin_l.weight, 1.0), (hp, p.lin_r.weight, 1.0)], p.lin_l.bias, True)
        saved.append((hu, hp, mean_d, mean_s, mean_e, w_root))
        hu, hp = hu_n, hp_n

    ls = link_structure(train_edge_index, interaction_type_tensor, num_users, n_p)
    if neg_ready is not None:
        torch.cuda.current_stream().wait_event(neg_ready)
    if neg_p.dtype != torch.int64 or neg_p.numel() != ls.n_edges:
        raise _lib.TrgError("neg_p must be int64 with one entry per positive edge (train_gnn.py:272)")
    if getattr(ls, "eid_long", None) is None:
        ls.eid_long = ls.by_user.eid.long()
    bu = ls.by_user
    col_neg64 = neg_p.index_select(0, ls.eid_long)
    neg_by_post = build_csr(ls.user_of_u, col_neg64, n_p, n_u, validate=False, per_step=True)
    neg_by_user = CSR(bu.rowptr, col_neg64.int(), bu.eid, bu.n_rows, bu.n_cols)
    l_pos, c_pos, dz_u = edge_anchor_loss(bu, hu, hp, ls.n_edges, 1, ls.wbar, True, None, coef_in_csr_order=True)
    l_neg, c_neg, dz_u = edge_anchor_loss(neg_by_user, hu, hp, ls.n_edges, 0, ls.wbar, True, dz_u,
                                          relu_gate=True, coef_in_csr_order=True)
    dz_p = gather_wsum(ls.by_post_u, c_pos, hu)
    gather_wsum(neg_by_post, c_neg, hu, out=dz_p, accumulate=True, relu_of=hp)
    del col_neg64
    loss = (l_pos + l_neg).reshape(())
    del neg_by_user, neg_by_post, c_pos, c_neg, hu, hp

    for li in range(len(layers) - 1, -1, -1):
        layer = layers[li]
        d, s, p = layer.msg_direct, layer.msg_social, layer.post_update
        wd, ws = float(layer.w_direct), float(layer.w_social)
        hu_in, hp_in, mean_d, mean_s, mean_e, w_root = saved.pop()
        (dw_d, dw_s, dw_root), db_u = sage_proj_bwd_weight(dz_u, [(mean_d, wd), (mean_s, ws), (hu_in, 1.0)], True)
        (dw_p, dw_pr), db_p = sage_proj_bwd_weight(dz_p, [(mean_e, 1.0), (hp_in, 1.0)], True)
        del mean_d, mean_s, mean_e
        _accum(d.lin_l.weight, dw_d)
        _accum(s.lin_l.weight, dw_s)
        _accum(d.lin_r.weight, wd * dw_root)
        _accum(s.lin_r.weight, ws * dw_root)
        _accum(d.lin_l.bias, wd * db_u)
        _accum(s.lin_l.bias, ws * db_u)
        _accum(p.lin_l.weight, dw_p)
        _accum(p.lin_r.weight, dw_pr)
        _accum(p.lin_l.bias, db_p)
        if li == 0:
            break
        g_md, g_ms, g_hu = sage_proj_bwd_input(
            dz_u, [(d.lin_l.weight, wd, rel_d.inv_deg), (s.lin_l.weight, ws, rel_s.inv_deg), (w_root, 1.0, None)])
        g_me, g_hp = sage_proj_bwd_input(dz_p, [(p.lin_l.weight, 1.0, rel_e.inv_deg), (p.lin_r.weight, 1.0, None)])
        del dz_u, dz_p
        sage_agg_bwd(rel_s.bwd, None, g_ms, out=g_hu, accumulate=True)
        sage_agg_bwd(rel_e.bwd, None, g_me, out=g_hu, accumulate=True, relu_of=hu_in)
        sage_agg_bwd(rel_d.bwd, None, g_md, out=g_hp, accumulate=True, relu_of=hp_in)
        dz_u, dz_p = g_hu, g_hp
    return loss
```

Baseline: 2.965 billion.

## Fuse negative-sample CSR build and post-side loss gradient into merged kernels

Replaces the per-step int64 index_select plus full CSR build for negative edges with a dedicated kernel that gathers negatives as int32, counts post degrees, and radix-sorts with an int32 key path. Positive and negative edges are merged into one by-post CSR. A new post-side edge kernel then recomputes the edge gradients directly instead of storing per-edge coefficients and running two gather_wsum passes. This cuts launches and coefficient traffic, at the cost of recomputing dot products on the post side and only applying when rows are 512 bytes wide.

```diff
diff --git a/include/trg_b200.h b/include/trg_b200.h
--- a/include/trg_b200.h
+++ b/include/trg_b200.h
@@ -8,7 +8,7 @@
 extern "C" {
 #endif
 
-#define TRG_ABI_VERSION 4
+#define TRG_ABI_VERSION 5
 
 enum { TRG_F32 = 0, TRG_BF16 = 1 };
 enum {
@@ -27,6 +27,13 @@
 int trg_csr_build(const int64_t* other, const int64_t* key, int64_t n_edges, int64_t n_key,
                   int32_t* rowptr , int32_t* col , int32_t* eid ,
                   void* workspace, size_t workspace_bytes, void* stream);
+
+size_t trg_loss_negatives_workspace_bytes(int64_t n_edges, int64_t n_posts);
+int trg_loss_negatives(const int64_t* neg_p, const int32_t* eid_u, const int32_t* user_of_u, int64_t n_edges,
+                       int64_t n_posts, const int32_t* rowptr_post, const int32_t* col_post,
+                       const int32_t* post_of_pos, const int32_t* rowptr_pos, const int32_t* vrow, int64_t n_rows,
+                       int32_t* col_neg , int32_t* rowptr_m , int32_t* col_m ,
+                       void* workspace, size_t workspace_bytes, void* stream);
 
 size_t trg_select_range_workspace_bytes(int64_t n);
 int trg_select_range(const int64_t* key, const int64_t* other, int64_t n, int64_t lo, int64_t hi,
@@ -81,6 +88,12 @@
                          const float* wbar, float* loss_out, float* coef_out, void* g_anchor,
                          int accumulate, int relu_gate, void* workspace, size_t workspace_bytes,
                          void* stream);
+
+int trg_edge_post_grad(const int32_t* rowptr, const int32_t* rowptr_pos, const int32_t* col, const int32_t* vrow,
+                       const int32_t* vinfo, const void* anchor, const void* gathered, int64_t n_rows,
+                       int64_t n_edges_scale, int32_t hidden, int dtype, const float* wbar, void* g_anchor,
+                       int relu_gate, const int32_t* long_rows, const int32_t* long_ptr, int64_t n_long,
+                       int64_t n_slots, float* partial, void* stream);
 
 typedef struct {
   const void* a;
diff --git a/truth_recommendation_gnn_b200/_lib.py b/truth_recommendation_gnn_b200/_lib.py
--- a/truth_recommendation_gnn_b200/_lib.py
+++ b/truth_recommendation_gnn_b200/_lib.py
@@ -9,7 +9,7 @@
 LIB_PATH = os.path.join(_HERE, "lib", "libtrg_b200.so")
 
 TRG_F32, TRG_BF16 = 0, 1
-ABI_VERSION = 4
+ABI_VERSION = 5
 
 _vp, _i64, _i32, _sz, _int = ctypes.c_void_p, ctypes.c_int64, ctypes.c_int32, ctypes.c_size_t, ctypes.c_int
 
@@ -37,6 +37,9 @@
     "trg_launch_count": (_i64, []),
     "trg_csr_workspace_bytes": (_sz, [_i64, _i64]),
     "trg_csr_build": (_int, [_vp, _vp, _i64, _i64, _vp, _vp, _vp, _vp, _sz, _vp]),
+    "trg_loss_negatives_workspace_bytes": (_sz, [_i64, _i64]),
+    "trg_loss_negatives": (_int, [_vp, _vp, _vp, _i64, _i64, _vp, _vp, _vp, _vp, _vp, _i64, _vp, _vp, _vp, _vp, _sz,
+                                  _vp]),
     "trg_select_range_workspace_bytes": (_sz, [_i64]),
     "trg_select_range": (_int, [_vp, _vp, _i64, _i64, _i64, _i64, _i64, _i64, _vp, _vp, _vp, _vp, _sz, _vp]),
     "trg_sage_agg_fwd": (_int, [_vp, _vp, _vp, _i64, _i32, _int, _vp, _vp, ctypes.POINTER(TrgLongRows), _vp]),
@@ -51,6 +54,8 @@
                                 _vp, _vp, _vp, _vp, _sz, _vp]),
     "trg_edge_anchor_loss": (_int, [_vp, _vp, _vp, _vp, _vp, _i64, _i64, _i32, _int, _int, _vp, _vp, _vp,
                                     _vp, _int, _int, _vp, _sz, _vp]),
+    "trg_edge_post_grad": (_int, [_vp, _vp, _vp, _vp, _vp, _vp, _vp, _i64, _i64, _i32, _int, _vp, _vp, _int, _vp,
+                                  _vp, _i64, _i64, _vp, _vp]),
     "trg_sage_proj_workspace_bytes": (_sz, [_i32, _i32, _int]),
     "trg_sage_proj_fwd": (_int, [ctypes.POINTER(TrgProjTerm), _i32, _vp, _i64, _i32, _int, _int, _vp,
                                  _vp, _sz, _vp]),
diff --git a/truth_recommendation_gnn_b200/csrc/csr_build.cu b/truth_recommendation_gnn_b200/csrc/csr_build.cu
--- a/truth_recommendation_gnn_b200/csrc/csr_build.cu
+++ b/truth_recommendation_gnn_b200/csrc/csr_build.cu
@@ -197,13 +197,15 @@
   asm volatile("ld.global.nc.L1::no_allocate.v2.u32 {%0,%1}, [%2];" : "=r"(r.x), "=r"(r.y) : "l"(p));
   return r;
 }
-template <bool FIRST>
+enum KeyIn { kKeyI64 = 0, kKeyI32 = 1, kPairs = 2 };
+template <int IN>
 __device__ __forceinline__ uint32_t load_key(const void* keys, int64_t idx) {
-  if (FIRST) return (uint32_t)ldg_stream(reinterpret_cast<const long long*>(keys) + idx);
+  if (IN == kKeyI64) return (uint32_t)ldg_stream(reinterpret_cast<const long long*>(keys) + idx);
+  if (IN == kKeyI32) return (uint32_t)ldg_stream(reinterpret_cast<const int*>(keys) + idx);
   return ldg_pair(reinterpret_cast<const uint2*>(keys) + idx).x;
 }
 
-template <bool FIRST>
+template <int IN>
 __global__ void __launch_bounds__(kThreads) radix_hist(const void* __restrict__ keys, int64_t n,
                                                        int shift, int* __restrict__ hist,
                                                        int n_ctas) {
@@ -214,16 +216,17 @@
 #pragma unroll
   for (int i = 0; i < kItems; ++i) {
     int64_t idx = base + (int64_t)i * kThreads + threadIdx.x;
-    if (idx < n) atomicAdd(&h[(load_key<FIRST>(keys, idx) >> shift) & (kRadix - 1)], 1);
+    if (idx < n) atomicAdd(&h[(load_key<IN>(keys, idx) >> shift) & (kRadix - 1)], 1);
   }
   __syncthreads();
   hist[(int64_t)threadIdx.x * n_ctas + blockIdx.x] = h[threadIdx.x];
 }
 
-template <bool FIRST, bool LAST>
+template <int IN, bool LAST>
 __global__ void __launch_bounds__(kThreads)
-    radix_scatter(const void* __restrict__ keys_in, int64_t n, int shift, const int* __restrict__ gbase,
-                  int n_ctas, uint2* __restrict__ pairs_out, uint32_t* __restrict__ vals_out) {
+    radix_scatter(const void* __restrict__ keys_in, const uint32_t* __restrict__ vals_in, int64_t n, int shift,
+                  const int* __restrict__ gbase, int n_ctas, uint2* __restrict__ pairs_out,
+                  uint32_t* __restrict__ vals_out, const int* __restrict__ out_off) {
   __shared__ int wcnt[kWarps][kRadix];
   __shared__ int sbase[kRadix];
   const int lane = threadIdx.x & 31, w = threadIdx.x >> 5;
@@ -236,9 +239,12 @@
   for (int r = 0; r < kItems; ++r) {
     int64_t idx = wbase + r * 32 + lane;
     bool valid = idx < n;
-    if (FIRST) {
-      key[r] = valid ? load_key<true>(keys_in, idx) : 0u;
+    if (IN == kKeyI64) {
+      key[r] = valid ? load_key<kKeyI64>(keys_in, idx) : 0u;
       val[r] = (uint32_t)idx;
+    } else if (IN == kKeyI32) {
+      key[r] = valid ? load_key<kKeyI32>(keys_in, idx) : 0u;
+      val[r] = valid ? (uint32_t)ldg_stream(reinterpret_cast<const int*>(vals_in) + idx) : 0u;
     } else {
       const uint2 kv = valid ? ldg_pair(reinterpret_cast<const uint2*>(keys_in) + idx) : make_uint2(0u, 0u);
       key[r] = kv.x;
@@ -277,7 +283,7 @@
       const int d = (int)((key[r] >> shift) & (kRadix - 1));
       const int dest = sbase[d] + wcnt[w][d] + rank[r];
       if (LAST)
-        vals_out[dest] = val[r];
+        vals_out[out_off ? __ldg(out_off + key[r] + 1) + dest : dest] = val[r];
       else
         pairs_out[dest] = make_uint2(key[r], val[r]);
     }
@@ -296,6 +302,38 @@
   int bits = 1;
   while (bits < 32 && ((int64_t)1 << bits) < n_key) ++bits;
   return (bits + 7) / 8;
+}
+
+__global__ void __launch_bounds__(kThreads) neg_gather_count(const long long* __restrict__ neg_p,
+                                                             const int* __restrict__ eid_u, int64_t n,
+                                                             long long n_key, int* __restrict__ col_neg,
+                                                             int* __restrict__ deg) {
+  int64_t i = (int64_t)blockIdx.x * blockDim.x + threadIdx.x;
+  const int64_t stride = (int64_t)gridDim.x * blockDim.x;
+  for (; i < n; i += stride) {
+    const long long k = neg_p[ldg_stream(eid_u + i)];
+    if ((unsigned long long)k >= (unsigned long long)n_key) {
+      printf("trg_loss_negatives: post id %lld of a negative (by-user edge %lld) is outside [0, %lld)\n", k,
+             (long long)i, n_key);
+      __trap();
+    }
+    col_neg[i] = (int)k;
+    atomicAdd(&deg[(int)k], 1);
+  }
+}
+
+__global__ void __launch_bounds__(kThreads)
+    merge_positives(const int* __restrict__ col_pos, const int* __restrict__ post_of_pos, int64_t n,
+                    const int* __restrict__ rp_neg, const int* __restrict__ rowptr_pos, const int* __restrict__ vrow,
+                    int64_t n_rows, int64_t n_key, int* __restrict__ col_m, int* __restrict__ rowptr_m) {
+  int64_t i = (int64_t)blockIdx.x * blockDim.x + threadIdx.x;
+  const int64_t stride = (int64_t)gridDim.x * blockDim.x;
+  for (int64_t j = i; j < n; j += stride)
+    col_m[j + __ldg(rp_neg + ldg_stream(post_of_pos + j))] = ldg_stream(col_pos + j);
+  for (int64_t v = i; v <= n_rows; v += stride) {
+    const int64_t row = v == n_rows ? n_key : (vrow ? (int64_t)__ldg(vrow + v) : v);
+    rowptr_m[v] = __ldg(rowptr_pos + v) + __ldg(rp_neg + row);
+  }
 }
 
 struct Workspace {
@@ -322,10 +360,92 @@
   return w;
 }
 
+int sort_pass(int in, bool last, const void* kin, const uint32_t* vin, int64_t e, int shift, const Workspace& w,
+              int n_ctas, uint2* kout, uint32_t* vout, const int* out_off, cudaStream_t st) {
+  if (in == kKeyI64)
+    radix_hist<kKeyI64><<<n_ctas, kThreads, 0, st>>>(kin, e, shift, w.hist, n_ctas);
+  else if (in == kKeyI32)
+    radix_hist<kKeyI32><<<n_ctas, kThreads, 0, st>>>(kin, e, shift, w.hist, n_ctas);
+  else
+    radix_hist<kPairs><<<n_ctas, kThreads, 0, st>>>(kin, e, shift, w.hist, n_ctas);
+  count_launch();
+  TRG_LAUNCH_OK();
+  int rc = exclusive_scan(w.hist, w.hist, (int64_t)kRadix * n_ctas, w.tile_sums, st);
+  if (rc) return rc;
+#define TRG_SCATTER(IN, LAST) \
+  radix_scatter<IN, LAST><<<n_ctas, kThreads, 0, st>>>(kin, vin, e, shift, w.hist, n_ctas, kout, vout, out_off)
+  if (in == kKeyI64) {
+    if (last) TRG_SCATTER(kKeyI64, true); else TRG_SCATTER(kKeyI64, false);
+  } else if (in == kKeyI32) {
+    if (last) TRG_SCATTER(kKeyI32, true); else TRG_SCATTER(kKeyI32, false);
+  } else {
+    if (last) TRG_SCATTER(kPairs, true); else TRG_SCATTER(kPairs, false);
+  }
+#undef TRG_SCATTER
+  count_launch();
+  TRG_LAUNCH_OK();
+  return TRG_OK;
+}
+
 }
 }
 
 using namespace trg;
+
+extern "C" size_t trg_loss_negatives_workspace_bytes(int64_t n_edges, int64_t n_posts) {
+  if (n_edges < 0 || n_posts < 0) return 0;
+  return carve(nullptr, n_edges, n_posts).bytes + align_up((size_t)(n_posts + 1) * 4, 256);
+}
+
+extern "C" int trg_loss_negatives(const int64_t* neg_p, const int32_t* eid_u, const int32_t* user_of_u,
+                                  int64_t n_edges, int64_t n_posts, const int32_t* rowptr_post,
+                                  const int32_t* col_post, const int32_t* post_of_pos, const int32_t* rowptr_pos,
+                                  const int32_t* vrow, int64_t n_rows, int32_t* col_neg, int32_t* rowptr_m,
+                                  int32_t* col_m, void* workspace, size_t workspace_bytes, void* stream) {
+  cudaStream_t st = reinterpret_cast<cudaStream_t>(stream);
+  const int64_t e = n_edges;
+  TRG_CHECK_ARG(e >= 0 && n_posts >= 0 && n_rows >= 0, "trg_loss_negatives: negative size");
+  TRG_CHECK_ARG(2 * e < ((int64_t)1 << 31) && n_posts < ((int64_t)1 << 31) - 1,
+                "trg_loss_negatives: 2 x %lld edges / %lld posts exceed int32 CSR range", (long long)e,
+                (long long)n_posts);
+  TRG_CHECK_ARG(rowptr_post && rowptr_pos && rowptr_m, "trg_loss_negatives: NULL row offsets");
+  TRG_CHECK_ARG(e == 0 || (neg_p && eid_u && user_of_u && col_post && post_of_pos && col_neg && col_m && n_posts > 0),
+                "trg_loss_negatives: NULL edge arrays with n_edges > 0");
+  Workspace w = carve(workspace, e, n_posts);
+  const size_t need = trg_loss_negatives_workspace_bytes(e, n_posts);
+  if (workspace == nullptr || workspace_bytes < need) {
+    set_error("trg_loss_negatives: workspace %zu < required %zu", workspace_bytes, need);
+    return TRG_E_WORKSPACE;
+  }
+  int* rp_neg = reinterpret_cast<int*>(reinterpret_cast<char*>(workspace) + w.bytes);
+  TRG_CUDA(cudaMemsetAsync(rp_neg, 0, (size_t)(n_posts + 1) * sizeof(int32_t), st));
+  const int grid_e = (int)std::max<int64_t>(ceil_div<int64_t>(e, kThreads), 1);
+  if (e > 0) {
+    neg_gather_count<<<grid_e, kThreads, 0, st>>>((const long long*)neg_p, eid_u, e, (long long)n_posts, col_neg,
+                                                   rp_neg);
+    count_launch();
+    TRG_LAUNCH_OK();
+    int rc = exclusive_scan(rp_neg, rp_neg, n_posts + 1, w.tile_sums, st);
+    if (rc) return rc;
+    const int passes = num_passes(n_posts);
+    const int n_ctas = (int)ceil_div<int64_t>(e, kTile);
+    const void* kin = col_neg;
+    for (int p = 0; p < passes; ++p) {
+      const bool first = p == 0, last = p == passes - 1;
+      uint2* kout = w.pairs[p & 1];
+      rc = sort_pass(first ? kKeyI32 : kPairs, last, kin, first ? (const uint32_t*)user_of_u : nullptr, e, 8 * p, w,
+                     n_ctas, kout, (uint32_t*)col_m, rowptr_post, st);
+      if (rc) return rc;
+      kin = kout;
+    }
+  }
+  const int grid_m = (int)std::max<int64_t>(ceil_div<int64_t>(std::max(e, n_rows + 1), kThreads), 1);
+  merge_positives<<<grid_m, kThreads, 0, st>>>(col_post, post_of_pos, e, rp_neg, rowptr_pos, vrow, n_rows, n_posts,
+                                               col_m, rowptr_m);
+  count_launch();
+  TRG_LAUNCH_OK();
+  return TRG_OK;
+}
 
 extern "C" size_t trg_csr_workspace_bytes(int64_t n_edges, int64_t n_key) {
   if (n_edges < 0 || n_key < 0) return 0;
@@ -371,24 +491,8 @@
     const int shift = 8 * p;
     uint2* kout = w.pairs[p & 1];
     uint32_t* vout = eid ? (uint32_t*)eid : w.vals;
-    if (first)
-      radix_hist<true><<<n_ctas, kThreads, 0, st>>>(kin, e, shift, w.hist, n_ctas);
-    else
-      radix_hist<false><<<n_ctas, kThreads, 0, st>>>(kin, e, shift, w.hist, n_ctas);
-    count_launch();
-    TRG_LAUNCH_OK();
-    int rc = exclusive_scan(w.hist, w.hist, (int64_t)kRadix * n_ctas, w.tile_sums, st);
+    int rc = sort_pass(first ? kKeyI64 : kPairs, last, kin, nullptr, e, shift, w, n_ctas, kout, vout, nullptr, st);
     if (rc) return rc;
-    if (first && last)
-      radix_scatter<true, true><<<n_ctas, kThreads, 0, st>>>(kin, e, shift, w.hist, n_ctas, kout, vout);
-    else if (first)
-      radix_scatter<true, false><<<n_ctas, kThreads, 0, st>>>(kin, e, shift, w.hist, n_ctas, kout, vout);
-    else if (last)
-      radix_scatter<false, true><<<n_ctas, kThreads, 0, st>>>(kin, e, shift, w.hist, n_ctas, kout, vout);
-    else
-      radix_scatter<false, false><<<n_ctas, kThreads, 0, st>>>(kin, e, shift, w.hist, n_ctas, kout, vout);
-    count_launch();
-    TRG_LAUNCH_OK();
     kin = kout;
     vin = vout;
   }
diff --git a/truth_recommendation_gnn_b200/csrc/edge_bce.cu b/truth_recommendation_gnn_b200/csrc/edge_bce.cu
--- a/truth_recommendation_gnn_b200/csrc/edge_bce.cu
+++ b/truth_recommendation_gnn_b200/csrc/edge_bce.cu
@@ -25,7 +25,18 @@
   int label;
   int accumulate;
   int relu_gate;
+  const int* rowptr_pos;
+  const int* vrow;
+  const int* vinfo;
+  float* partial;
+  int64_t n_slots;
 };
+
+template <typename T>
+__device__ __forceinline__ float round_to(float x) {
+  if constexpr (sizeof(T) == 2) return __bfloat162float(__float2bfloat16_rn(x));
+  return x;
+}
 
 __device__ __forceinline__ float softplus(float x) {
   return fmaxf(x, 0.f) + log1pf(expf(-fabsf(x)));
@@ -35,17 +46,19 @@
   return x >= 0.f ? __fdiv_rn(1.f, 1.f + e) : __fdiv_rn(e, 1.f + e);
 }
 
-template <typename T, int LPR, int VPL, int R, bool TWO>
-__global__ void __launch_bounds__(kThreads, VPL == 1 ? 3 : 2) edge_bce(const BceArgs a) {
+template <typename T, int LPR, int VPL, int R, bool TWO, bool POST = false>
+__global__ void __launch_bounds__(kThreads, VPL == 1 && !(POST && sizeof(T) == 2) ? 3 : 2) edge_bce(const BceArgs a) {
   constexpr int kVec = Elem<T>::kVec;
   constexpr int kUnroll = (LPR < 8 ? (LPR >= 4 ? 2 : 1) : (VPL == 1 ? 4 : 2)) * (TWO ? 1 : 2);
   static_assert(R < LPR, "row boundaries are held one per lane");
+  static_assert(!(TWO && POST), "the post-side mode gathers one row per edge");
   __shared__ double red[2][kThreads / 32];
   const int lane = threadIdx.x & 31;
   const int gl = lane & (LPR - 1);
   const unsigned gmask = LPR == 32 ? 0xffffffffu : (((1u << LPR) - 1u) << (lane & ~(LPR - 1)));
   const int64_t r0 = ((int64_t)blockIdx.x * (kThreads / LPR) + threadIdx.x / LPR) * R;
   const bool want_grad = a.g_u != nullptr;
+  const bool want_coef = !POST && a.c_pos != nullptr;
   float sp_sum = 0.f, sn_sum = 0.f;
 
   if (r0 < a.n_users) {
@@ -57,26 +70,71 @@
     const char* pb = reinterpret_cast<const char*>(a.p);
     const char* ub = reinterpret_cast<const char*>(a.u);
     const float wbar = __ldg(a.wbar);
+    int my_pp = 0, my_vrow = 0, my_vinfo = 0;
+    if (POST) {
+      const int rr = min(gl, nr - 1);
+      my_pp = ldg_stream(a.rowptr_pos + r0 + min(gl, nr));
+      my_vrow = a.vrow ? __ldg(a.vrow + r0 + rr) : (int)(r0 + rr);
+      my_vinfo = a.vinfo ? __ldg(a.vinfo + r0 + rr) : 0;
+    }
+    auto arow = [&](int c) -> int64_t { return POST ? (int64_t)__shfl_sync(gmask, my_vrow, c, LPR) : r0 + c; };
+    auto neg_start = [&](int c) -> int {
+      return POST ? __shfl_sync(gmask, my_ptr, c, LPR) + __shfl_sync(gmask, my_pp, c + 1, LPR) -
+                        __shfl_sync(gmask, my_pp, c, LPR)
+                  : 0;
+    };
 
     bool act[VPL];
-    float uf[VPL][kVec], ga[VPL][kVec];
+    float uf[VPL][kVec], ga[VPL][kVec], gn[VPL][kVec];
     uint4 u_nxt[VPL];
+    const int64_t ar0 = arow(0), ar1 = arow(min(1, nr - 1));
 #pragma unroll
     for (int i = 0; i < VPL; ++i) {
       act[i] = gl + i * LPR < a.row_vecs;
 #pragma unroll
-      for (int k = 0; k < kVec; ++k) uf[i][k] = ga[i][k] = 0.f;
+      for (int k = 0; k < kVec; ++k) uf[i][k] = ga[i][k] = gn[i][k] = 0.f;
       u_nxt[i] = make_uint4(0, 0, 0, 0);
       if (act[i]) {
-        Elem<T>::unpack(ldg_row(ub + (size_t)r0 * row_bytes + (size_t)(gl + i * LPR) * 16), uf[i]);
-        if (nr > 1) u_nxt[i] = ldg_row(ub + (size_t)(r0 + 1) * row_bytes + (size_t)(gl + i * LPR) * 16);
+        Elem<T>::unpack(ldg_row(ub + (size_t)ar0 * row_bytes + (size_t)(gl + i * LPR) * 16), uf[i]);
+        if (nr > 1) u_nxt[i] = ldg_row(ub + (size_t)ar1 * row_bytes + (size_t)(gl + i * LPR) * 16);
       }
     }
     int cur = 0;
     int cur_end = __shfl_sync(gmask, my_ptr, 1, LPR);
+    int neg_beg = neg_start(0);
 
     auto flush = [&]() {
-      if (want_grad) {
+      if (POST) {
+        const int info = __shfl_sync(gmask, my_vinfo, cur, LPR);
+        const int64_t orow = arow(cur);
+        if (a.vinfo && info < 0) {
+          const size_t feat = (size_t)a.row_vecs * kVec;
+          float* pp = a.partial + (size_t)(-(info + 1)) * feat;
+          float* pn = pp + (size_t)a.n_slots * feat;
+#pragma unroll
+          for (int i = 0; i < VPL; ++i)
+            if (act[i]) {
+#pragma unroll
+              for (int k = 0; k < kVec; ++k) {
+                pp[(size_t)(gl + i * LPR) * kVec + k] = ga[i][k];
+                pn[(size_t)(gl + i * LPR) * kVec + k] = gn[i][k];
+              }
+            }
+        } else {
+          char* ob = reinterpret_cast<char*>(a.g_u) + (size_t)orow * row_bytes;
+#pragma unroll
+          for (int i = 0; i < VPL; ++i)
+            if (act[i]) {
+              float f[kVec];
+#pragma unroll
+              for (int k = 0; k < kVec; ++k) {
+                f[k] = gn[i][k] + round_to<T>(ga[i][k]);
+                if (a.relu_gate) f[k] = uf[i][k] > 0.f ? f[k] : 0.f;
+              }
+              stg_stream(ob + (size_t)(gl + i * LPR) * 16, Elem<T>::pack(f));
+            }
+        }
+      } else if (want_grad) {
         char* ob = reinterpret_cast<char*>(a.g_u) + (size_t)(r0 + cur) * row_bytes;
 #pragma unroll
         for (int i = 0; i < VPL; ++i)
@@ -96,13 +154,15 @@
       }
       ++cur;
       cur_end = __shfl_sync(gmask, my_ptr, min(cur + 1, nr), LPR);
+      neg_beg = neg_start(min(cur, nr - 1));
+      const int64_t an = arow(min(cur + 1, nr - 1));
 #pragma unroll
       for (int i = 0; i < VPL; ++i) {
         Elem<T>::unpack(u_nxt[i], uf[i]);
 #pragma unroll
-        for (int k = 0; k < kVec; ++k) ga[i][k] = 0.f;
+        for (int k = 0; k < kVec; ++k) ga[i][k] = gn[i][k] = 0.f;
         if (act[i] && cur + 1 < nr)
-          u_nxt[i] = ldg_row(ub + (size_t)(r0 + cur + 1) * row_bytes + (size_t)(gl + i * LPR) * 16);
+          u_nxt[i] = ldg_row(ub + (size_t)an * row_bytes + (size_t)(gl + i * LPR) * 16);
       }
     };
 
@@ -192,11 +252,13 @@
         }
         constexpr int kLanesPerVal = LPR / NV;
         const int j = gl / kLanesPerVal;
-        const bool is_neg = TWO ? (j & 1) : (a.label == 0);
+        const bool is_neg = TWO ? (j & 1) : (POST ? e0 + t + j >= neg_beg : a.label == 0);
         const float z = is_neg ? v[0] : -v[0];
-        const float spv = softplus(z);
-        if ((gl % kLanesPerVal) == 0 && (TWO ? (j >> 1) : j) < bsz) {
-          if (is_neg) sn_sum += spv; else sp_sum += spv;
+        if (!POST) {
+          const float spv = softplus(z);
+          if ((gl % kLanesPerVal) == 0 && (TWO ? (j >> 1) : j) < bsz) {
+            if (is_neg) sn_sum += spv; else sp_sum += spv;
+          }
         }
         if (want_grad) {
           const float coef = (is_neg ? 1.f : -wbar) * sigmoid(z) * a.inv_e;
@@ -209,6 +271,7 @@
                 my_cpos = cpos;
                 my_cneg = cneg;
               }
+              const bool to_neg = POST && e0 + t + q >= neg_beg;
 #pragma unroll
               for (int i = 0; i < VPL; ++i)
                 if (act[i]) {
@@ -216,15 +279,18 @@
                   Elem<T>::unpack(vp[q][i], fp);
                   if (TWO) Elem<T>::unpack(vn[q][i], fn);
 #pragma unroll
-                  for (int k = 0; k < kVec; ++k)
-                    ga[i][k] = TWO ? fmaf(cpos, fp[k], fmaf(cneg, fn[k], ga[i][k])) : fmaf(cpos, fp[k], ga[i][k]);
+                  for (int k = 0; k < kVec; ++k) {
+                    if (TWO) ga[i][k] = fmaf(cpos, fp[k], fmaf(cneg, fn[k], ga[i][k]));
+                    else if (to_neg) gn[i][k] = fmaf(cpos, fp[k], gn[i][k]);
+                    else ga[i][k] = fmaf(cpos, fp[k], ga[i][k]);
+                  }
                 }
             }
           }
         }
         t += bsz;
       }
-      if (want_grad && e0 + gl < e_end) {
+      if (want_coef && e0 + gl < e_end) {
         a.c_pos[id_cur] = my_cpos;
         if (TWO) a.c_neg[id_cur] = my_cneg;
       }
@@ -234,6 +300,7 @@
     }
     while (cur < nr) flush();
   }
+  if (POST) return;
 
   double dsp = sp_sum, dsn = sn_sum;
 #pragma unroll
@@ -276,10 +343,11 @@
 constexpr int kRingS = 16;
 constexpr int kRingBytes = (kThreads / 32) * kRingS * 512;
 
-template <typename T>
-__global__ void __launch_bounds__(kThreads, 3) edge_anchor_ring(const BceArgs a) {
+template <typename T, bool POST = false, int R = 4>
+__global__ void __launch_bounds__(kThreads, POST && sizeof(T) == 2 ? 2 : 3) edge_anchor_ring(const BceArgs a) {
   constexpr int kVec = Elem<T>::kVec;
-  constexpr int R = 4, G = kRingG, S = kRingS;
+  constexpr int G = kRingG, S = kRingS;
+  static_assert(R < 32, "row boundaries are held one per lane");
   constexpr unsigned full = 0xffffffffu;
   extern __shared__ __align__(16) unsigned char ring_raw[];
   __shared__ double red[2][kThreads / 32];
@@ -288,6 +356,7 @@
                           (uint32_t)(warp * S * 512 + lane * 16);
   const int64_t r0 = ((int64_t)blockIdx.x * (kThreads / 32) + warp) * R;
   const bool want_grad = a.g_u != nullptr;
+  const bool want_coef = !POST && a.c_pos != nullptr;
   float s_sum = 0.f;
 
   if (r0 < a.n_users) {
@@ -299,18 +368,51 @@
     const char* ub = reinterpret_cast<const char*>(a.u);
     const float wbar = __ldg(a.wbar);
     const bool is_neg = a.label == 0;
-
-    float uf[kVec], ga[kVec];
+    int my_pp = 0, my_vrow = 0, my_vinfo = 0;
+    if (POST) {
+      const int rr = min(lane, nr - 1);
+      my_pp = ldg_stream(a.rowptr_pos + r0 + min(lane, nr));
+      my_vrow = a.vrow ? __ldg(a.vrow + r0 + rr) : (int)(r0 + rr);
+      my_vinfo = a.vinfo ? __ldg(a.vinfo + r0 + rr) : 0;
+    }
+    auto arow = [&](int c) -> int64_t { return POST ? (int64_t)__shfl_sync(full, my_vrow, c) : r0 + c; };
+    auto neg_start = [&](int c) -> int {
+      return POST ? __shfl_sync(full, my_ptr, c) + __shfl_sync(full, my_pp, c + 1) - __shfl_sync(full, my_pp, c) : 0;
+    };
+
+    float uf[kVec], ga[kVec], gn[kVec];
     uint4 u_nxt = make_uint4(0, 0, 0, 0);
 #pragma unroll
-    for (int k = 0; k < kVec; ++k) ga[k] = 0.f;
-    Elem<T>::unpack(ldg_row(ub + (size_t)r0 * 512 + (size_t)lane * 16), uf);
-    if (nr > 1) u_nxt = ldg_row(ub + (size_t)(r0 + 1) * 512 + (size_t)lane * 16);
+    for (int k = 0; k < kVec; ++k) ga[k] = gn[k] = 0.f;
+    const int64_t ar0 = arow(0), ar1 = arow(min(1, nr - 1));
+    Elem<T>::unpack(ldg_row(ub + (size_t)ar0 * 512 + (size_t)lane * 16), uf);
+    if (nr > 1) u_nxt = ldg_row(ub + (size_t)ar1 * 512 + (size_t)lane * 16);
     int cur = 0;
     int cur_end = __shfl_sync(full, my_ptr, 1);
+    int neg_beg = neg_start(0);
 
     auto flush = [&]() {
-      if (want_grad) {
+      if (POST) {
+        const int info = __shfl_sync(full, my_vinfo, cur);
+        const int64_t orow = arow(cur);
+        if (a.vinfo && info < 0) {
+          float* pp = a.partial + (size_t)(-(info + 1)) * (32 * kVec) + (size_t)lane * kVec;
+          float* pn = pp + (size_t)a.n_slots * (32 * kVec);
+#pragma unroll
+          for (int k = 0; k < kVec; ++k) {
+            pp[k] = ga[k];
+            pn[k] = gn[k];
+          }
+        } else {
+          float f[kVec];
+#pragma unroll
+          for (int k = 0; k < kVec; ++k) {
+            f[k] = gn[k] + round_to<T>(ga[k]);
+            if (a.relu_gate) f[k] = uf[k] > 0.f ? f[k] : 0.f;
+          }
+          stg_stream(reinterpret_cast<char*>(a.g_u) + (size_t)orow * 512 + (size_t)lane * 16, Elem<T>::pack(f));
+        }
+      } else if (want_grad) {
         char* ob = reinterpret_cast<char*>(a.g_u) + (size_t)(r0 + cur) * 512 + (size_t)lane * 16;
         if (a.accumulate) {
           float f[kVec];
@@ -326,10 +428,12 @@
       }
       ++cur;
       cur_end = __shfl_sync(full, my_ptr, min(cur + 1, nr));
+      neg_beg = neg_start(min(cur, nr - 1));
+      const int64_t an = arow(min(cur + 1, nr - 1));
       Elem<T>::unpack(u_nxt, uf);
 #pragma unroll
-      for (int k = 0; k < kVec; ++k) ga[k] = 0.f;
-      if (cur + 1 < nr) u_nxt = ldg_row(ub + (size_t)(r0 + cur + 1) * 512 + (size_t)lane * 16);
+      for (int k = 0; k < kVec; ++k) ga[k] = gn[k] = 0.f;
+      if (cur + 1 < nr) u_nxt = ldg_row(ub + (size_t)an * 512 + (size_t)lane * 16);
     };
     auto load_id = [&](int ebase) -> int {
       const int e = ebase + lane;
@@ -355,7 +459,7 @@
     for (int e_base = e_beg; e_base < e_end; e_base += G) {
       const int cnt = min(G, e_end - e_base);
       int my_id = 0;
-      if (want_grad && lane < cnt) my_id = a.eid ? ldg_stream(a.eid + e_base + lane) : e_base + lane;
+      if (want_coef && lane < cnt) my_id = a.eid ? ldg_stream(a.eid + e_base + lane) : e_base + lane;
       cp_async_wait<1>();
       __syncwarp();
       float my_c = 0.f;
@@ -397,26 +501,33 @@
         }
         constexpr int kLanesPerVal = 32 / G;
         const int j = lane / kLanesPerVal;
-        const float z = is_neg ? v[0] : -v[0];
-        const float spv = softplus(z);
-        if ((lane % kLanesPerVal) == 0 && j < bsz) s_sum += spv;
+        const bool neg_j = POST ? e_base + t + j >= neg_beg : is_neg;
+        const float z = neg_j ? v[0] : -v[0];
+        if (!POST) {
+          const float spv = softplus(z);
+          if ((lane % kLanesPerVal) == 0 && j < bsz) s_sum += spv;
+        }
         if (want_grad) {
-          const float coef = (is_neg ? 1.f : -wbar) * sigmoid(z) * a.inv_e;
+          const float coef = (neg_j ? 1.f : -wbar) * sigmoid(z) * a.inv_e;
 #pragma unroll
           for (int q = 0; q < G; ++q) {
             const float cq = __shfl_sync(full, coef, q * kLanesPerVal);
             if (q < bsz) {
               if (lane == t + q) my_c = cq;
+              const bool to_neg = POST && e_base + t + q >= neg_beg;
               float fp[kVec];
               Elem<T>::unpack(vp[q], fp);
 #pragma unroll
-              for (int k = 0; k < kVec; ++k) ga[k] = fmaf(cq, fp[k], ga[k]);
+              for (int k = 0; k < kVec; ++k) {
+                if (to_neg) gn[k] = fmaf(cq, fp[k], gn[k]);
+                else ga[k] = fmaf(cq, fp[k], ga[k]);
+              }
             }
           }
         }
         t += bsz;
       }
-      if (want_grad && lane < cnt) a.c_pos[my_id] = my_c;
+      if (want_coef && lane < cnt) a.c_pos[my_id] = my_c;
       __syncwarp();
       const int nid_next = load_id(e_base + 3 * G);
       issue(e_base + 2 * G, nid, slot);
@@ -426,6 +537,7 @@
     while (cur < nr) flush();
     cp_async_wait<0>();
   }
+  if (POST) return;
 
   double dsum = s_sum;
 #pragma unroll
@@ -473,14 +585,33 @@
   }
 }
 
-template <typename T, bool TWO>
+template <typename T>
+__global__ void __launch_bounds__(128) post_combine_long(const BceArgs a, const int* __restrict__ long_rows,
+                                                         const int* __restrict__ long_ptr) {
+  const int i = blockIdx.x;
+  const int64_t orow = long_rows[i];
+  const int s0 = long_ptr[i], s1 = long_ptr[i + 1];
+  const int feat = a.row_vecs * Elem<T>::kVec;
+  const T* anchor = reinterpret_cast<const T*>(a.u) + (size_t)orow * feat;
+  T* out = reinterpret_cast<T*>(a.g_u) + (size_t)orow * feat;
+  const float* neg = a.partial + ((size_t)a.n_slots + s1 - 1) * feat;
+  for (int f = threadIdx.x; f < feat; f += blockDim.x) {
+    float s = 0.f;
+    for (int sl = s0; sl < s1; ++sl) s += a.partial[(size_t)sl * feat + f];
+    float v = neg[f] + round_to<T>(s);
+    if (a.relu_gate && !((float)anchor[f] > 0.f)) v = 0.f;
+    out[f] = (T)v;
+  }
+}
+
+template <typename T, bool TWO, bool POST = false>
 int launch_bce(BceArgs& a, int64_t* n_blocks_out, cudaStream_t st, bool dry) {
   const int rv = a.row_vecs;
-#define TRG_BCE_CASE(LPR, VPL, R)                                                     \
-  {                                                                                   \
-    const int64_t grid = ceil_div<int64_t>(a.n_users, (int64_t)(kThreads / LPR) * R); \
-    *n_blocks_out = grid;                                                             \
-    if (!dry) edge_bce<T, LPR, VPL, R, TWO><<<(unsigned)grid, kThreads, 0, st>>>(a);  \
+#define TRG_BCE_CASE(LPR, VPL, R)                                                           \
+  {                                                                                         \
+    const int64_t grid = ceil_div<int64_t>(a.n_users, (int64_t)(kThreads / LPR) * R);       \
+    *n_blocks_out = grid;                                                                   \
+    if (!dry) edge_bce<T, LPR, VPL, R, TWO, POST><<<(unsigned)grid, kThreads, 0, st>>>(a);  \
   }
   if (rv <= 2) TRG_BCE_CASE(2, 1, 1)
   else if (rv <= 4) TRG_BCE_CASE(4, 1, 2)
@@ -560,8 +691,7 @@
   cudaStream_t st = reinterpret_cast<cudaStream_t>(stream);
   TRG_CHECK_ARG(n_rows >= 0 && n_edges_scale >= 0, "trg_edge_anchor_loss: negative size");
   TRG_CHECK_ARG(loss_out && wbar, "trg_edge_anchor_loss: NULL loss_out/wbar");
-  TRG_CHECK_ARG((coef_out == nullptr) == (g_anchor == nullptr),
-                "trg_edge_anchor_loss: coef_out and g_anchor must be both NULL or both non-NULL");
+  TRG_CHECK_ARG(coef_out == nullptr || g_anchor != nullptr, "trg_edge_anchor_loss: coef_out needs g_anchor");
   TRG_CHECK_ARG(n_rows == 0 || (rowptr && anchor), "trg_edge_anchor_loss: NULL rowptr / anchor table");
   TRG_CHECK_ARG(((uintptr_t)anchor | (uintptr_t)gathered | (uintptr_t)g_anchor) % 16 == 0,
                 "trg_edge_anchor_loss: tables must be 16-byte aligned");
@@ -609,3 +739,62 @@
   TRG_LAUNCH_OK();
   return TRG_OK;
 }
+
+#ifndef TRG_POST_ROWS
+#define TRG_POST_ROWS 16
+#endif
+constexpr int kPostRows = TRG_POST_ROWS;
+
+extern "C" int trg_edge_post_grad(const int32_t* rowptr, const int32_t* rowptr_pos, const int32_t* col,
+                                  const int32_t* vrow, const int32_t* vinfo, const void* anchor, const void* gathered,
+                                  int64_t n_rows, int64_t n_edges_scale, int32_t hidden, int dtype, const float* wbar,
+                                  void* g_anchor, int relu_gate, const int32_t* long_rows, const int32_t* long_ptr,
+                                  int64_t n_long, int64_t n_slots, float* partial, void* stream) {
+  cudaStream_t st = reinterpret_cast<cudaStream_t>(stream);
+  TRG_CHECK_ARG(n_rows >= 0 && n_edges_scale >= 0 && n_long >= 0 && n_slots >= 0, "trg_edge_post_grad: negative size");
+  TRG_CHECK_ARG(wbar && g_anchor, "trg_edge_post_grad: NULL wbar / g_anchor");
+  TRG_CHECK_ARG(n_rows == 0 || (rowptr && rowptr_pos && anchor), "trg_edge_post_grad: NULL rowptr / anchor table");
+  TRG_CHECK_ARG(((uintptr_t)anchor | (uintptr_t)gathered | (uintptr_t)g_anchor) % 16 == 0,
+                "trg_edge_post_grad: tables must be 16-byte aligned");
+  TRG_CHECK_ARG(dtype == TRG_F32 || dtype == TRG_BF16, "trg_edge_post_grad: unknown dtype %d", dtype);
+  TRG_CHECK_ARG((vinfo == nullptr) == (n_long == 0) && (n_long == 0 || (vrow && long_rows && long_ptr && partial)),
+                "trg_edge_post_grad: slices of long rows need vrow, vinfo, long_rows, long_ptr and partial");
+  const int es = dtype == TRG_BF16 ? 2 : 4;
+  TRG_CHECK_ARG(hidden > 0 && (hidden * es) % 16 == 0,
+                "trg_edge_post_grad: row width %d x %d bytes is not a multiple of 16 bytes", hidden, es);
+  BceArgs a{};
+  a.rowptr = rowptr; a.col_p = col; a.u = anchor; a.p = gathered; a.wbar = wbar; a.g_u = g_anchor;
+  a.n_users = n_rows;
+  a.inv_e = n_edges_scale > 0 ? (float)(1.0 / (double)n_edges_scale) : 0.f;
+  a.row_vecs = hidden * es / 16;
+  a.relu_gate = relu_gate ? 1 : 0;
+  a.rowptr_pos = rowptr_pos; a.vrow = vrow; a.vinfo = vinfo; a.partial = partial; a.n_slots = n_slots;
+  if (n_rows == 0) return TRG_OK;
+  if (a.row_vecs == 32 && !anchor_ring_off()) {
+    const int64_t n_blocks = ceil_div<int64_t>(n_rows, (int64_t)(kThreads / 32) * kPostRows);
+    static SmemAttrState attr_f32, attr_bf16;
+    if (dtype == TRG_F32) {
+      TRG_CUDA(ensure_dyn_smem(edge_anchor_ring<float, true, kPostRows>, kRingBytes, attr_f32));
+      edge_anchor_ring<float, true, kPostRows><<<(unsigned)n_blocks, kThreads, kRingBytes, st>>>(a);
+    } else {
+      TRG_CUDA(ensure_dyn_smem(edge_anchor_ring<__nv_bfloat16, true, kPostRows>, kRingBytes, attr_bf16));
+      edge_anchor_ring<__nv_bfloat16, true, kPostRows><<<(unsigned)n_blocks, kThreads, kRingBytes, st>>>(a);
+    }
+  } else {
+    int64_t n_blocks = 0;
+    int rc = dtype == TRG_F32 ? launch_bce<float, false, true>(a, &n_blocks, st, false)
+                              : launch_bce<__nv_bfloat16, false, true>(a, &n_blocks, st, false);
+    if (rc) return rc;
+  }
+  count_launch();
+  TRG_LAUNCH_OK();
+  if (n_long > 0) {
+    if (dtype == TRG_F32)
+      post_combine_long<float><<<(unsigned)n_long, 128, 0, st>>>(a, long_rows, long_ptr);
+    else
+      post_combine_long<__nv_bfloat16><<<(unsigned)n_long, 128, 0, st>>>(a, long_rows, long_ptr);
+    count_launch();
+    TRG_LAUNCH_OK();
+  }
+  return TRG_OK;
+}
diff --git a/truth_recommendation_gnn_b200/functional.py b/truth_recommendation_gnn_b200/functional.py
--- a/truth_recommendation_gnn_b200/functional.py
+++ b/truth_recommendation_gnn_b200/functional.py
@@ -182,14 +182,30 @@
         self.n_edges = int(pos_u.numel())
         self.by_user = build_csr(pos_p, pos_u, self.num_users, self.num_posts)
         self.by_post = build_csr(pos_u, pos_p, self.num_posts, self.num_users, validate=False)
+        self._user_of_u = None
+        self._post_of_pos = None
+        self._post_rows = {}
         self._by_post_u = None
-        self._user_of_u = None
+        self._user_of_u64 = None
+        self._eid_long = None
         if self.n_edges:
             w = interaction_type_tensor[pos_p + num_users].float()
             self.wbar = w.mean().reshape(1).contiguous()
         else:
             self.wbar = torch.full((1,), float("nan"), device=pos_u.device)
 
+
+    @staticmethod
+    def _expand_rows(csr: CSR) -> torch.Tensor:
+        rp = csr.rowptr.long()
+        return torch.repeat_interleave(torch.arange(csr.n_rows, device=rp.device, dtype=torch.int32),
+                                       rp[1:] - rp[:-1]).contiguous()
+
+    @property
+    def user_of_u(self) -> torch.Tensor:
+        if self._user_of_u is None:
+            self._user_of_u = self._expand_rows(self.by_user)
+        return self._user_of_u
 
     @property
     def by_post_u(self) -> CSR:
@@ -201,12 +217,40 @@
         return self._by_post_u
 
     @property
-    def user_of_u(self) -> torch.Tensor:
-        if self._user_of_u is None:
-            rp = self.by_user.rowptr.long()
-            self._user_of_u = torch.repeat_interleave(
-                torch.arange(self.num_users, device=rp.device), rp[1:] - rp[:-1]).contiguous()
-        return self._user_of_u
+    def user_of_u64(self) -> torch.Tensor:
+        if self._user_of_u64 is None:
+            self._user_of_u64 = self.user_of_u.long()
+        return self._user_of_u64
+
+    @property
+    def eid_long(self) -> torch.Tensor:
+        if self._eid_long is None:
+            self._eid_long = self.by_user.eid.long()
+        return self._eid_long
+
+    @property
+    def post_of_pos(self) -> torch.Tensor:
+        if self._post_of_pos is None:
+            self._post_of_pos = self._expand_rows(self.by_post)
+        return self._post_of_pos
+
+    def post_rows(self, row_bytes: int):
+        split = row_bytes >= 80
+        if split not in self._post_rows:
+            bp = self.by_post
+            lr = bp.long_rows() if split else None
+            if lr is None:
+                self._post_rows[split] = (bp.rowptr, None, None)
+            else:
+                rp = bp.rowptr.long()
+                deg = rp[1:] - rp[:-1]
+                t = int(lr.vrowptr.numel() - 1)
+                counts = torch.ones_like(deg)
+                counts[lr.long_rows.long()] = lr.long_ptr[1:].long() - lr.long_ptr[:-1].long()
+                vrow = torch.repeat_interleave(torch.arange(bp.n_rows, device=rp.device, dtype=torch.int32), counts)
+                assert vrow.numel() == t
+                self._post_rows[split] = (lr.vrowptr, vrow.contiguous(), lr)
+        return self._post_rows[split]
 
 
 _LINK_CACHE: dict = {}
@@ -257,7 +301,7 @@
 
 
 def edge_anchor_loss(csr: CSR, anchor, gathered, n_edges_scale, label, wbar, want_grad, g_anchor=None,
-                     relu_gate=False, coef_in_csr_order=False):
+                     relu_gate=False, coef_in_csr_order=False, want_coef=True):
     lib = _lib.load()
     anchor, gathered = anchor.contiguous(), gathered.contiguous()
     _check_rows(anchor, "edge_anchor_loss")
@@ -266,7 +310,8 @@
     coef = None
     accumulate = g_anchor is not None
     if want_grad:
-        coef = torch.empty(csr.n_edges, dtype=torch.float32, device=dev)
+        if want_coef:
+            coef = torch.empty(csr.n_edges, dtype=torch.float32, device=dev)
         if g_anchor is None:
             g_anchor = torch.empty_like(anchor)
     else:
@@ -275,10 +320,10 @@
     ws = torch.empty(ws_bytes, dtype=torch.uint8, device=dev)
     e = csr.n_edges
     rb = anchor.size(1) * anchor.element_size()
-    nbytes = e * (rb + 12) + csr.n_rows * (rb * (2 if want_grad else 1) + 4)
+    nbytes = e * (rb + (12 if coef is not None else 4)) + csr.n_rows * (rb * (2 if want_grad else 1) + 4)
     _lib.call("trg_edge_anchor_loss", nbytes, lib.trg_edge_anchor_loss,
               _lib.ptr(csr.rowptr), _lib.ptr(csr.col) if e else None,
-              _lib.ptr(csr.eid) if (e and not coef_in_csr_order) else None,
+              _lib.ptr(csr.eid) if (e and coef is not None and not coef_in_csr_order) else None,
               _lib.ptr(anchor), _lib.ptr(gathered), csr.n_rows, int(n_edges_scale), anchor.size(1),
               _lib.dtype_code(anchor.dtype), 1 if label else 0, _lib.ptr(wbar), _lib.ptr(loss), _lib.ptr(coef),
               _lib.ptr(g_anchor), 1 if (accumulate and want_grad) else 0,
@@ -286,6 +331,58 @@
     return loss, coef, g_anchor
 
 
+def loss_negatives(ls: LinkStructure, neg_p, row_bytes: int):
+    lib = _lib.load()
+    if neg_p.dtype != torch.int64 or neg_p.numel() != ls.n_edges:
+        raise _lib.TrgError("neg_p must be int64 with one entry per positive edge (train_gnn.py:272)")
+    neg_p = neg_p.contiguous()
+    bu, bp = ls.by_user, ls.by_post
+    e, n_p = ls.n_edges, ls.num_posts
+    rowptr_pos, vrow, lr = ls.post_rows(row_bytes)
+    n_rows = int(rowptr_pos.numel()) - 1
+    dev = neg_p.device
+    col_neg = torch.empty(e, dtype=torch.int32, device=dev)
+    col_m = torch.empty(2 * e, dtype=torch.int32, device=dev)
+    rowptr_m = torch.empty(n_rows + 1, dtype=torch.int32, device=dev)
+    ws_bytes = int(lib.trg_loss_negatives_workspace_bytes(e, n_p))
+    ws = torch.empty(ws_bytes, dtype=torch.uint8, device=dev)
+    nbytes = e * (20 + 3 * 16 + 4 + 16) + 4 * (3 * n_p + 2 * n_rows)
+    _lib.call("trg_loss_negatives", nbytes, lib.trg_loss_negatives,
+              _lib.ptr(neg_p) if e else None, _lib.ptr(bu.eid) if e else None, _lib.ptr(ls.user_of_u) if e else None,
+              e, n_p, _lib.ptr(bp.rowptr), _lib.ptr(bp.col) if e else None, _lib.ptr(ls.post_of_pos) if e else None,
+              _lib.ptr(rowptr_pos), _lib.ptr(vrow), n_rows, _lib.ptr(col_neg) if e else None, _lib.ptr(rowptr_m),
+              _lib.ptr(col_m) if e else None, _lib.ptr(ws), ws_bytes, _lib.stream())
+    return CSR(bu.rowptr, col_neg, bu.eid, bu.n_rows, bu.n_cols), (rowptr_m, rowptr_pos, col_m, vrow, lr)
+
+
+def edge_post_grad(ls: LinkStructure, rows, post_emb, user_emb, n_edges_scale, relu_gate=True):
+    lib = _lib.load()
+    rowptr_m, rowptr_pos, col_m, vrow, lr = rows
+    post_emb, user_emb = post_emb.contiguous(), user_emb.contiguous()
+    _check_rows(post_emb, "edge_post_grad")
+    if post_emb.dtype != user_emb.dtype or post_emb.size(1) != user_emb.size(1):
+        raise _lib.TrgError("user and post embeddings must share dtype and width")
+    feat = post_emb.size(1)
+    out = torch.empty_like(post_emb)
+    n_rows = int(rowptr_m.numel()) - 1
+    partial = n_long = n_slots = None
+    if lr is not None:
+        n_slots = lr.n_slots
+        n_long = int(lr.long_rows.numel())
+        partial = torch.empty(2 * n_slots, feat, dtype=torch.float32, device=post_emb.device)
+    e2 = int(col_m.numel())
+    rb = feat * post_emb.element_size()
+    nbytes = e2 * (rb + 4) + ls.num_posts * 2 * rb + 8 * (n_rows + 1)
+    _lib.call("trg_edge_post_grad", nbytes, lib.trg_edge_post_grad,
+              _lib.ptr(rowptr_m), _lib.ptr(rowptr_pos), _lib.ptr(col_m) if e2 else None, _lib.ptr(vrow),
+              _lib.ptr(lr.vinfo) if lr is not None else None, _lib.ptr(post_emb), _lib.ptr(user_emb), n_rows,
+              int(n_edges_scale), feat, _lib.dtype_code(post_emb.dtype), _lib.ptr(ls.wbar), _lib.ptr(out),
+              1 if relu_gate else 0, _lib.ptr(lr.long_rows) if lr is not None else None,
+              _lib.ptr(lr.long_ptr) if lr is not None else None, n_long or 0, n_slots or 0, _lib.ptr(partial),
+              _lib.stream())
+    return out
+
+
 class LinkBCEFn(torch.autograd.Function):
 
     @staticmethod
@@ -293,8 +390,6 @@
         want = user_emb.requires_grad or post_emb.requires_grad
         if neg_p.dtype != torch.int64 or neg_p.numel() != ls.n_edges:
             raise _lib.TrgError("neg_p must be int64 with one entry per positive edge (train_gnn.py:272)")
-        if getattr(ls, "eid_long", None) is None:
-            ls.eid_long = ls.by_user.eid.long()
         e_scale = int(getattr(ls, "n_edges_scale", ls.n_edges))
         bu = ls.by_user
         ctx.neg_by_post = None
diff --git a/truth_recommendation_gnn_b200/fused_step.py b/truth_recommendation_gnn_b200/fused_step.py
--- a/truth_recommendation_gnn_b200/fused_step.py
+++ b/truth_recommendation_gnn_b200/fused_step.py
@@ -3,8 +3,8 @@
 import torch
 
 from . import _lib
-from .functional import (edge_anchor_loss, gather_wsum, link_structure, sage_agg_bwd, sage_agg_fwd,
-                         sage_proj_bwd_input, sage_proj_bwd_weight, sage_proj_fwd)
+from .functional import (edge_anchor_loss, edge_post_grad, gather_wsum, link_structure, loss_negatives,
+                         sage_agg_bwd, sage_agg_fwd, sage_proj_bwd_input, sage_proj_bwd_weight, sage_proj_fwd)
 from .graph import CSR, build_csr, relation_graph
 from .nn import REL_DIRECT, REL_ENGAGE, REL_SOCIAL, StackedWeightedRGCN, WeightedRGCN
 
@@ -78,22 +78,29 @@
     ls = link_structure(train_edge_index, interaction_type_tensor, num_users, n_p)
     if neg_ready is not None:
         torch.cuda.current_stream().wait_event(neg_ready)
-    if neg_p.dtype != torch.int64 or neg_p.numel() != ls.n_edges:
-        raise _lib.TrgError("neg_p must be int64 with one entry per positive edge (train_gnn.py:272)")
-    if getattr(ls, "eid_long", None) is None:
-        ls.eid_long = ls.by_user.eid.long()
-    bu = ls.by_user
-    col_neg64 = neg_p.index_select(0, ls.eid_long)
-    neg_by_post = build_csr(ls.user_of_u, col_neg64, n_p, n_u, validate=False, per_step=True)
-    neg_by_user = CSR(bu.rowptr, col_neg64.int(), bu.eid, bu.n_rows, bu.n_cols)
-    l_pos, c_pos, dz_u = edge_anchor_loss(bu, hu, hp, ls.n_edges, 1, ls.wbar, True, None, coef_in_csr_order=True)
-    l_neg, c_neg, dz_u = edge_anchor_loss(neg_by_user, hu, hp, ls.n_edges, 0, ls.wbar, True, dz_u,
-                                          relu_gate=True, coef_in_csr_order=True)
-    dz_p = gather_wsum(ls.by_post_u, c_pos, hu)
-    gather_wsum(neg_by_post, c_neg, hu, out=dz_p, accumulate=True, relu_of=hp)
-    del col_neg64
+    if hp.size(1) * hp.element_size() == 512:
+        neg_by_user, post_rows = loss_negatives(ls, neg_p, 512)
+        l_pos, _, dz_u = edge_anchor_loss(ls.by_user, hu, hp, ls.n_edges, 1, ls.wbar, True, None, want_coef=False)
+        l_neg, _, dz_u = edge_anchor_loss(neg_by_user, hu, hp, ls.n_edges, 0, ls.wbar, True, dz_u, relu_gate=True,
+                                          want_coef=False)
+        dz_p = edge_post_grad(ls, post_rows, hp, hu, ls.n_edges)
+        del neg_by_user, post_rows
+    else:
+        if neg_p.dtype != torch.int64 or neg_p.numel() != ls.n_edges:
+            raise _lib.TrgError("neg_p must be int64 with one entry per positive edge (train_gnn.py:272)")
+        bu = ls.by_user
+        col_neg64 = neg_p.index_select(0, ls.eid_long)
+        neg_by_post = build_csr(ls.user_of_u64, col_neg64, n_p, n_u, validate=False, per_step=True)
+        neg_by_user = CSR(bu.rowptr, col_neg64.int(), bu.eid, bu.n_rows, bu.n_cols)
+        del col_neg64
+        l_pos, c_pos, dz_u = edge_anchor_loss(bu, hu, hp, ls.n_edges, 1, ls.wbar, True, None, coef_in_csr_order=True)
+        l_neg, c_neg, dz_u = edge_anchor_loss(neg_by_user, hu, hp, ls.n_edges, 0, ls.wbar, True, dz_u,
+                                              relu_gate=True, coef_in_csr_order=True)
+        dz_p = gather_wsum(ls.by_post_u, c_pos, hu)
+        gather_wsum(neg_by_post, c_neg, hu, out=dz_p, accumulate=True, relu_of=hp)
+        del neg_by_user, neg_by_post, c_pos, c_neg
     loss = (l_pos + l_neg).reshape(())
-    del neg_by_user, neg_by_post, c_pos, c_neg, hu, hp
+    del hu, hp
 
     for li in range(len(layers) - 1, -1, -1):
         layer = layers[li]
```

After: 3.022 billion, median of 6. 1.9% higher.
